# google-research/corenet

Hardware: AMD Instinct MI355X
Metric: voxels/sec fwd+bwd @128^3 (higher is better)
Workload: dtype bf16x3 (the convolutions of decoder stages 3-6 and the encoder's 3x3 convolutions -- forward of stages 4-5, data gradient of all -- multiply operands split into two bf16 terms: three bf16 MFMAs per product, fp32 accumulation, 16 mantissa bits, ~3e-6 relative per layer; tensors, everything else and t

## Files before the change

corenet_amd/_lib.py:

```python
from __future__ import annotations

import ctypes as C
import os
from typing import Optional

import torch as t

_HERE = os.path.dirname(os.path.abspath(__file__))
TOOLS_LIB_PATH = os.path.join(os.path.dirname(_HERE), "tools", "_build", "libcorenet_hip_tools.so")
PROBE_LIB_PATH = os.path.join(os.path.dirname(_HERE), "tools", "_build", "libcrn_probe.so")
LIB_PATH = os.environ.get("CORENET_HIP_LIB", TOOLS_LIB_PATH if os.environ.get("CRN_TOOLS_LIB") == "1" else
                          os.path.join(_HERE, "lib", "libcorenet_hip.so"))

c_i32p = C.POINTER(C.c_int32)
c_f32p = C.c_void_p
vp = C.c_void_p
i64 = C.c_int64
i32 = C.c_int
f32 = C.c_float
sz = C.c_size_t


class CrnTapBoxes(C.Structure):
  _fields_ = [("n_groups", C.c_int32), ("c_groups", C.c_int32), ("n_box", (C.c_int8 * 6) * 8),
# ... 53 lines not shown
                         C.POINTER(CrnView), i32, i32, i32, i32, i32, i32, i32, vp, vp],
    "crn_conv_fwd_bf3_slabs": [C.POINTER(CrnView), C.POINTER(CrnInTransform), vp, i32, vp, i32,
                               C.POINTER(CrnView), i32, i32, i32, i32, i32, i32, i32, vp, vp],
    "crn_conv_fwd_bf3_slabs_bnbwd": [C.POINTER(CrnView), C.POINTER(CrnInTransform), vp, i32, vp, i32,
                                     C.POINTER(CrnView), i32, i32, i32, i32, i32, i32, i32, vp, C.POINTER(CrnBnBwdFuse), vp],
    "crn_conv_fwd_bf3_slabs_stats": [C.POINTER(CrnView), C.POINTER(CrnInTransform), vp, i32, vp, i32,
                                     C.POINTER(CrnView), i32, i32, i32, i32, i32, i32, i32, vp, i32, vp, sz, C.POINTER(C.c_int), vp],
    "crn_batch_renorm_bwd_apply": [vp, i64, vp, i64, i32, i32, i64, i32, vp, vp, vp, vp, vp, i64, vp, vp, i32, vp, i32,
                                   vp, sz, i32, vp],
    "crn_conv_wgrad_bf3": [C.POINTER(CrnView), C.POINTER(CrnInTransform), C.POINTER(CrnView), vp, i32,
                           i32, i32, i32, i32, i32, i32, i32, vp],
    "crn_conv_wgrad_bf3_boxes": [C.POINTER(CrnView), C.POINTER(CrnInTransform), C.POINTER(CrnView), vp, i32,
                                 i32, i32, i32, i32, i32, i32, i32, vp, vp],
    "crn_conv_fwd_bf3_plan": [C.POINTER(CrnView), C.POINTER(CrnInTransform), vp, vp, i32, vp, i32,
                              C.POINTER(CrnView), i32, i32, i32, i32, i32, i32, i32, vp, vp, vp],
    "crn_conv_wgrad_bf3_plan": [C.POINTER(CrnView), C.POINTER(CrnInTransform), C.POINTER(CrnView), vp, i32,
                                i32, i32, i32, i32, i32, i32, i32, vp, vp],
    "crn_conv_wgrad": [C.POINTER(CrnView), C.POINTER(CrnInTransform), C.POINTER(CrnView), vp, i32,
                       i32, i32, i32, i32, i32, i32, i32, vp, vp],
    "crn_bf3_operands": [vp, vp, i32, i64, vp, vp],
    "crn_bf3_gather_image": [vp, vp, i32, vp, vp],
    "crn_convt_s2k7_fwd_bf3": [vp, i64, i32, i32, i32, i32, C.POINTER(CrnInTransform), vp, vp, vp, i64, i64, i32, vp],
    "crn_convt_s2k7_dgrad_bf3": [vp, i64, i64, i32, i32, i32, i32, i32, vp, vp, i64, i32, vp],
    "crn_convt_s2k7_c2_fwd_bf3": [vp, i64, i32, i32, i32, i32, C.POINTER(CrnInTransform), vp, vp, vp, i64, i64, i32, vp],
    "crn_convt_s2k7_c2_dgrad_bf3": [vp, i64, i64, i32, i32, i32, i32, i32, vp, vp, i64, i32, vp],
    "crn_convt_s2k7_wgrad_bf3": [vp, i64, i32, i32, i32, i32, C.POINTER(CrnInTransform), vp, i64, i64, i32, vp, i32, i32, vp, vp],
    "crn_convt_s2k7_ximage": [vp, i64, i32, i32, i32, i32, C.POINTER(CrnInTransform), vp, sz, vp],
    "crn_splitk_defer": [i32],
    "crn_splitk_reserve": [i64, vp],
    "crn_splitk_release": [vp],
    "crn_set_deterministic": [i32],
    "crn_roctx_push": [C.c_char_p],
    "crn_roctx_pop": [],
    "crn_comm_unique_id": [vp],
    "crn_comm_init": [vp, i32, i32, C.POINTER(vp)],
    "crn_comm_destroy": [vp],
    "crn_comm_info": [vp, C.POINTER(i32), C.POINTER(i32), C.POINTER(i32)],
    "crn_allreduce_f32": [vp, vp, i64, vp],
    "crn_broadcast_f32": [vp, vp, i64, i32, vp],
    "crn_conv_wgrad_1x1_bf3": [C.POINTER(CrnView), C.POINTER(CrnInTransform), C.POINTER(CrnView), vp, i32, i32, vp],
    "crn_conv_wgrad_2d_bf3": [C.POINTER(CrnView), C.POINTER(CrnInTransform), C.POINTER(CrnView), vp, i32, i32, i32, i32,
                              i32, i32, vp],
    "crn_conv2d_bf3": [C.POINTER(CrnView), C.POINTER(CrnInTransform), vp, i32, vp, i32, C.POINTER(CrnView),
                       i32, i32, i32, i32, i32, vp],
    "crn_conv2d_bf3_plan": [C.POINTER(CrnView), C.POINTER(CrnInTransform), vp, i32, vp, i32, C.POINTER(CrnView),
                            i32, i32, i32, i32, i32, vp],
    "crn_conv_wgrad_2d_bf3_plan": [C.POINTER(CrnView), C.POINTER(CrnInTransform), C.POINTER(CrnView), vp, i32, i32, i32, i32,
                                   i32, i32, vp],
    "crn_copy_tiles_f32": [vp, vp, vp, vp, vp, i64, i32, vp],
    "crn_copy_mats_f32": [vp, vp, vp, i64, i32, vp],
    "crn_gather_f32": [vp, vp, vp, i64, vp],
    "crn_scatter_f32": [vp, vp, vp, i64, i32, vp],
    "crn_bias_grad": [vp, i32, i32, i64, i64, vp, i32, vp, sz, vp],
    "crn_batch_renorm_stats": [vp, i32, i32, i64, i64, i32, vp, vp, vp, vp, vp, f32, f32, i32,
                               vp, vp, vp, vp, sz, vp],
    "crn_batch_renorm_stats_tail": [vp, i32, i32, i64, i64, vp, vp, vp, vp, vp, f32, f32, i32, vp, vp, vp, vp, sz,
                                    vp, vp, vp, i64, vp, i64, vp, i64, i32, vp, i32, vp],
    "crn_batch_renorm_bwd_head": [vp, i64, vp, i64, vp, i64, vp, i64, vp, i64, i32, i32, i64, vp, vp, vp, vp, vp, i64,
                                  vp, vp, i32, vp, i32, vp, sz, vp, i32, vp],
    "crn_batch_renorm_bwd": [vp, i64, vp, i64, i32, i32, i64, i32, i32, vp, vp, vp, vp, vp, i64,
                             vp, vp, i32, vp, i32, vp, sz, vp],
    "crn_affine_add_relu": [vp, vp, vp, vp, vp, vp, i32, i32, i64, i64, i64, vp, i64, vp, i64, i32, vp],
    "crn_relu_bwd_add": [vp, vp, vp, i32, i32, i64, i64, i64, i64, vp, i64, vp],
    "crn_preprocess_caffe": [vp, i32, i32, i32, vp, vp],
    "crn_stem_conv_fwd": [vp, i32, i32, i32, vp, vp, vp, vp, sz, vp],
    "crn_stem_conv_wgrad": [vp, i32, i32, i32, vp, vp, vp],
    "crn_batch_renorm_finalize": [vp, i32, i32, C.c_double, vp, vp, vp, vp, vp, f32, f32, vp, vp, vp, vp],
    "crn_bn_relu_maxpool_fwd": [vp, vp, vp, i32, i32, i32, i32, vp, vp, vp],
    "crn_bn_relu_maxpool_bwd": [vp, vp, i32, i32, i32, i32, vp, vp],
    "crn_relu_mean_fwd": [vp, i32, i32, i64, i64, vp, vp],
    "crn_relu_mean_bwd": [vp, vp, i32, i32, i64, i64, vp, i64, i32, vp],
    "crn_linear_fwd": [vp, vp, vp, i32, i32, i32, vp, i32, vp],
    "crn_linear_bwd": [vp, vp, vp, i32, i32, i32, i32, vp, vp, vp, vp],
    "crn_stride2_gather": [vp, vp, i32, i32, i32, i32, i32, i32, vp],
    "crn_stride2_scatter": [vp, vp, i32, i32, i32, i32, i32, i32, vp],
    "crn_fill_offset_channels": [vp, i32, i64, i64, i32, vp, vp],
    "crn_decoder_inputs": [vp, vp, i32, i32, C.POINTER(C.c_float), vp, vp, vp],
    "crn_ray_sample_fwd": [vp, i64, i64, i64, i32, i32, i32, i32, vp, vp, vp, i64, i32, i32, i32, vp],
    "crn_ray_sample_bwd": [vp, i64, i32, i32, i32, i32, i32, vp, vp, vp, i64, i32, i32, i32, vp],
    "crn_ray_sample_fwd_idx": [vp, i64, i64, i64, i32, i32, i32, i32, vp, vp, vp, i64, i32, i32, i32, vp, vp],
    "crn_ray_project": [vp, vp, i32, i32, i32, i32, i32, i32, vp, vp],
    "crn_ray_sample_bwd_idx": [vp, i64, i32, i32, i32, i32, i32, vp, vp, i64, i32, i32, i32, vp],
    "crn_loss_fwd_bwd": [i32, vp, vp, vp, i32, i32, i64, vp, vp, f32, vp, sz, vp],
    "crn_argmax_confusion": [vp, vp, i32, i32, i64, vp, vp, vp],
    "crn_softmax_superres": [vp, i32, i32, i32, i32, i32, i32, vp, vp],
    "crn_eval_labels": [vp, vp, vp, i32, i32, i32, i32, i32, i32, i32, i32, vp, vp, vp, vp],
    "crn_eval_labels_cpu": [vp, vp, vp, i32, i32, i32, i32, i32, i32, i32, i32, vp, vp, vp, i32],
    "crn_eval_scores_tiles": [vp],
    "crn_eval_scores": [vp, i32, vp, vp, i32, i32, i32, i32, i32, i32, i32, i32, i32, vp, vp, vp, vp],
    "crn_eval_scores_cpu": [vp, i32, vp, vp, i32, i32, i32, i32, i32, i32, i32, i32, i32, vp, vp, vp, i32],
    "crn_score_softmax": [vp, i32, i32, i64, vp, vp],
    "crn_score_softmax_cpu": [vp, i32, i32, i64, vp, i32],
    "crn_adam_step": [vp, vp, vp, vp, i64, f32, f32, f32, f32, f32, i32, vp],
    "crn_adam_set_hyper": [vp, f32, f32, f32, f32, f32, i32, vp],
    "crn_adam_step_hyper": [vp, vp, vp, vp, i64, vp, vp],
    "crn_fill_voxels": [vp, vp, i32, i32, i32, i32, i32, vp, sz, vp],
    "crn_fill_voxels_strided": [vp, C.POINTER(i64), vp, C.POINTER(i64), i32, i32, i32, i32, i32, vp, sz, vp],
    "crn_fill_voxels_cpu": [vp, vp, i32, i32, i32, i32, i32, i32],
    "crn_marching_cubes_count": [vp, C.POINTER(i64), i32, i32, i32, i32, f32, vp, sz, vp, vp],
    "crn_marching_cubes_emit": [vp, C.POINTER(i64), i32, i32, i32, i32, f32, vp, vp, sz, vp, vp, vp, vp],
    "crn_marching_cubes_cpu": [vp, C.POINTER(i64), i32, i32, i32, i32, f32, vp, vp, vp, vp, vp, i32],
    "crn_box_filter": [vp, C.POINTER(i64), vp, i32, i32, i32, i32, i32, vp, sz, vp],
    "crn_box_filter_cpu": [vp, C.POINTER(i64), vp, i32, i32, i32, i32, i32, i32],
    "crn_render_bin": [vp, vp, i32, i32, i32, i32, i64, vp, vp, vp, vp],
    "crn_render_raster": [vp, vp, vp, vp, i32, vp, i32, i32, i32, i32, vp, vp, vp, vp, vp, vp],
    "crn_render_cpu": [vp, vp, vp, vp, i32, vp, i32, i32, i32, vp, i32],
    "crn_render_raster_tex": [vp, vp, vp, vp, i32, vp, i32, i32, i32, i32, vp, vp, vp, vp, vp, vp, vp, vp, i32, i32, i32, vp],
    "crn_render_cpu_tex": [vp, vp, vp, vp, i32, vp, i32, i32, i32, vp, vp, vp, vp, i32, i32, i32, i32],
    "crn_render_raster_geometry": [vp, vp, i32, i32, i32, i32, vp, vp, vp, vp, vp, vp, vp, vp, vp],
    "crn_render_cpu_geometry": [vp, vp, i32, i32, i32, vp, vp, vp, vp, i32],
    "crn_voxel_faces_count": [vp, i32, i32, i32, i32, vp, i32, vp, vp, vp, sz, vp, vp],
    "crn_voxel_faces_emit": [vp, i32, i32, i32, i32, vp, i32, vp, i32, vp, sz, vp, vp, vp, vp],
    "crn_voxel_faces_cpu": [vp, i32, i32, i32, i32, vp, i32, vp, vp, vp, i32, vp, vp, vp, vp, i32],
    "crn_sample_surface": [vp, vp, i32, i64, i64, C.c_uint32, vp, sz, vp, vp, vp, vp],
    "crn_sample_surface_cpu": [vp, vp, i32, i64, C.c_uint32, vp, vp, vp, i32],
    "crn_nearest": [vp, vp, vp, vp, i32, i64, i64, i64, vp, sz, vp, vp, vp],
    "crn_nearest_cpu": [vp, vp, vp, vp, i32, vp, vp, i32],
    "crn_point_triangle": [vp, vp, vp, vp, i32, i64, i64, i64, i64, vp, sz, vp, vp, vp],
    "crn_point_triangle_cpu": [vp, vp, vp, vp, i32, vp, vp, i32],
    "crn_voxel_components_bricks": [vp],
    "crn_voxel_components": [vp, C.POINTER(i64), i32, i32, i32, i32, i32, i32, i32, vp, sz, vp, vp, vp],
    "crn_component_stats": [vp, vp, C.POINTER(i64), i32, i32, i32, i32, i32, vp, i64, vp, vp, vp, vp, vp],
    "crn_voxel_components_cpu": [vp, C.POINTER(i64), i32, i32, i32, i32, i32, i32, i32, vp, vp, i32],
    "crn_component_stats_cpu": [vp, vp, C.POINTER(i64), i32, i32, i32, i32, i32, vp, i64, vp, vp, vp, vp, i32],
    "crn_voxel_distance_tiles": [vp],
    "crn_voxel_distance": [vp, C.POINTER(i64), i32, i32, i32, i32, i32, i32, vp, sz, vp, vp, vp],
    "crn_voxel_distance_cpu": [vp, C.POINTER(i64), i32, i32, i32, i32, i32, i32, vp, vp, i32],
    "crn_voxel_visibility_tiles": [vp],
    "crn_voxel_visibility": [vp, C.POINTER(i64), i32, i32, i32, i32, i32, vp, i32, vp, sz, vp, vp, vp],
    "crn_voxel_visibility_cpu": [vp, C.POINTER(i64), i32, i32, i32, i32, i32, vp, i32, vp, vp, i32],
    "crn_voxel_overlap_tiles": [vp],
    "crn_voxel_overlap": [vp, C.POINTER(i64), i32, vp, C.POINTER(i64), i32, i32, i32, i32, i32, vp, vp, vp, vp, sz, vp, vp],
    "crn_voxel_overlap_cpu": [vp, C.POINTER(i64), i32, vp, C.POINTER(i64), i32, i32, i32, i32, i32, vp, vp, vp, vp, vp, i32],
    "crn_voxel_topology_tiles": [vp],
    "crn_voxel_topology": [vp, C.POINTER(i64), i32, i32, i32, i32, i32, i32, i32, vp, vp, vp],
    "crn_voxel_topology_cpu": [vp, C.POINTER(i64), i32, i32, i32, i32, i32, i32, i32, vp, vp, i32],
    "crn_mesh_tiles": [vp],
    "crn_mesh_corner_count": [vp, i64, vp, vp, i32, i64, vp, vp, vp],
    "crn_mesh_corner_lists": [vp, i64, vp, vp, i32, i64, vp, vp, vp, vp, vp, vp, vp, vp, vp],
    "crn_mesh_neighbours": [vp, vp, vp, i64, vp, vp],
    "crn_mesh_smooth_step": [vp, vp, vp, vp, vp, f32, i64, vp],
    "crn_mesh_face_normals": [vp, vp, i64, vp, vp, i32, i64, vp, vp],
    "crn_mesh_vertex_normals": [vp, vp, i64, vp, i32, i64, vp, vp, vp, vp],
    "crn_mesh_cluster_build": [vp, i64, vp, i64, vp, vp, i32, f32, vp, vp, i32, vp, vp, vp, vp, vp],
    "crn_mesh_cluster_emit": [vp, i64, vp, i64, vp, vp, i32, f32, vp, vp, vp, vp, vp, vp, vp, i64, i64, vp, vp, vp, vp, vp, vp],
    "crn_mesh_topology_cpu": [vp, i64, vp, vp, i32, i64, vp, vp, vp, vp, vp, vp],
    "crn_mesh_smooth_step_cpu": [vp, vp, vp, vp, vp, f32, i64],
    "crn_mesh_face_normals_cpu": [vp, vp, i64, vp, vp, i32, i64, vp],
    "crn_mesh_vertex_normals_cpu": [vp, vp, i64, vp, i32, i64, vp, vp, vp],
    "crn_mesh_cluster_cpu": [vp, i64, vp, i64, vp, vp, i32, f32, vp, vp, vp, vp, vp],
    "crn_voxelize_mesh": [vp, vp, i32, vp, i32, i32, i32, i32, i32, f32, i32, i32, vp, vp],
    "crn_batch_renorm_eval_affine": [vp, vp, vp, i32, f32, vp, vp, vp],
    "crn_transform_meshes": [vp, vp, i32, vp, i32, vp, vp],
    "crn_merge_labels": [vp, vp, vp, i32, i32, i32, i32, i32, vp, vp],
    "crn_zero_f32": [vp, i64, vp],
    "crn_add_i64": [vp, i32, i64, vp],
}
_SIZE_FNS = {
    "crn_batch_renorm_workspace_bytes": [i32],
    "crn_loss_workspace_bytes": [i32, i32],
    "crn_fill_voxels_workspace_bytes": [i32, i32, i32, i32],
    "crn_marching_cubes_workspace_bytes": [i32, i32, i32, i32],
    "crn_voxel_faces_workspace_bytes": [i32, i32, i32, i32],
    "crn_sample_surface_workspace_bytes": [i64, i32],
    "crn_nearest_workspace_bytes": [i64],
    "crn_point_triangle_workspace_bytes": [i64, i64],
# ... 130 lines not shown
```

corenet_amd/backend.py:

```python
from __future__ import annotations

import ctypes as C
from typing import Optional

import torch as t

from corenet_amd import _lib
from corenet_amd._lib import CrnInTransform, CrnView, ptr
from corenet_amd.views import View, space_to_depth_view, view_of

_DTYPE_CODE = {t.float32: 0, t.uint8: 1, t.int32: 2, t.float64: 3, t.int64: 4, t.int16: 5, t.int8: 6}


def _cview(v: View) -> CrnView:
  base = v.storage.data_ptr() + 4 * (v.offset - v.storage.storage_offset())
  c = v.__dict__.get("_crn")
  if c is None or c[0] != base:
    c = (base, CrnView(base, v.B, v.C, v.D, v.H, v.W, v.sB, v.sC, ptr(v.chan_off), v.sD, v.sH, v.sW))
    object.__setattr__(v, "_crn", c)
  return c[1]


class Transform:
  __slots__ = ("scale", "shift", "pre_relu", "post_relu")
# ... 279 lines not shown

  def bn_stats(self, x: t.Tensor, B, Cn, S, sB, pre_relu, gamma, beta, rmean, rvar, nbt, eps,
               momentum, training, scale, shift, saved):
    ws, n = self._bn_ws(Cn, x.device)
    self.lib.crn_batch_renorm_stats(ptr(x), B, Cn, S, sB, int(pre_relu), ptr(gamma), ptr(beta),
                                    ptr(rmean), ptr(rvar), ptr(nbt), eps, momentum, int(training),
                                    ptr(scale), ptr(shift), ptr(saved), ptr(ws), n, _lib.stream())

  def stem_conv_fwd(self, img: t.Tensor, w_packed: t.Tensor, bias, y: t.Tensor, stats: bool) -> int:
    B, _, H, W = img.shape
    parts = int(self.lib.crn_stem_conv_parts(B, H, W)) if stats else 0
    ws, n = self._bn_ws(64, img.device) if stats else (None, 0)
    self.lib.crn_stem_conv_fwd(ptr(img), B, H, W, ptr(w_packed), ptr(bias), ptr(y), ptr(ws), n, _lib.stream())
    return parts

  def bn_finalize(self, parts: int, Cn: int, count: float, gamma, beta, rmean, rvar, nbt, eps, momentum, scale, shift, saved):
    ws, _ = self._bn_ws(Cn, scale.device)
    self.lib.crn_batch_renorm_finalize(ptr(ws), parts, Cn, float(count), ptr(gamma), ptr(beta), ptr(rmean), ptr(rvar),
                                       ptr(nbt), eps, momentum, ptr(scale), ptr(shift), ptr(saved), _lib.stream())

  def bn_stats_tail(self, x, B, Cn, S, sB, gamma, beta, rmean, rvar, nbt, eps, momentum, training, scale, shift, saved,
                    r, rscale, rshift, sB_r, y_pre, sB_pre, y, sB_y, relu, y2=None, W=0):
    ws, n = self._bn_ws(Cn, x.device)
    self.lib.crn_batch_renorm_stats_tail(ptr(x), B, Cn, S, sB, ptr(gamma), ptr(beta), ptr(rmean), ptr(rvar), ptr(nbt),
                                         eps, momentum, int(training), ptr(scale), ptr(shift), ptr(saved), ptr(ws), n,
                                         ptr(r), ptr(rscale), ptr(rshift), sB_r, ptr(y_pre), sB_pre, ptr(y), sB_y,
                                         int(relu), ptr(y2), int(W), _lib.stream())

  def bn_bwd(self, x, sB_x, dy, sB_dy, B, Cn, S, pre_relu, post_relu, gamma, scale, shift, saved,
             dx, sB_dx, dgamma, dbeta, accumulate=False, dsum=None, ndsum=0):
    ws, n = self._bn_ws(Cn, x.device)
    self.lib.crn_batch_renorm_bwd(ptr(x), sB_x, ptr(dy), sB_dy, B, Cn, S, int(pre_relu),
                                  int(post_relu), ptr(gamma), ptr(scale), ptr(shift), ptr(saved),
                                  ptr(dx), sB_dx, ptr(dgamma), ptr(dbeta), int(accumulate),
                                  ptr(dsum), int(ndsum), ptr(ws), n, _lib.stream())

  def bn_bwd_head(self, x, sB_x, dy, sB_dy, g, sB_g, act, sB_act, g2, sB_g2, B, Cn, S, gamma, scale, shift, saved,
                  dx, sB_dx, dgamma, dbeta, accumulate=False, dsum=None, ndsum=0, g_compact=None, W=0):
    ws, n = self._bn_ws(Cn, x.device)
    self.lib.crn_batch_renorm_bwd_head(ptr(x), sB_x, ptr(dy), sB_dy, ptr(g), sB_g, ptr(act), sB_act, ptr(g2), sB_g2,
                                       B, Cn, S, ptr(gamma), ptr(scale), ptr(shift), ptr(saved), ptr(dx), sB_dx,
                                       ptr(dgamma), ptr(dbeta), int(accumulate), ptr(dsum), int(ndsum), ptr(ws), n,
                                       ptr(g_compact), int(W), _lib.stream())

  def bn_eval_affine(self, params, buffers, table, eps, scale, shift):
    self.lib.crn_batch_renorm_eval_affine(ptr(params), ptr(buffers), ptr(table), table.shape[0], eps,
                                          ptr(scale), ptr(shift), _lib.stream())

  def affine_add_relu(self, x, scale, shift, r, rscale, rshift, B, Cn, S, sB_x, sB_r,
                      y_pre, sB_pre, y, sB_y, relu):
    self.lib.crn_affine_add_relu(ptr(x), ptr(scale), ptr(shift), ptr(r), ptr(rscale), ptr(rshift),
                                 B, Cn, S, sB_x, sB_r, ptr(y_pre), sB_pre, ptr(y), sB_y, int(relu),
                                 _lib.stream())

  def relu_bwd_add(self, dy, y_pre, dy2, B, Cn, S, sB_dy, sB_pre, sB_dy2, dx, sB_dx):
    self.lib.crn_relu_bwd_add(ptr(dy), ptr(y_pre), ptr(dy2), B, Cn, S, sB_dy, sB_pre, sB_dy2,
                              ptr(dx), sB_dx, _lib.stream())

  def preprocess(self, img_u8, out):
    B, _, H, W = img_u8.shape
    self.lib.crn_preprocess_caffe(ptr(img_u8), B, H, W, ptr(out), _lib.stream())

  def maxpool_fwd(self, x, scale, shift, B, Cn, H, W, y, argmax):
    self.lib.crn_bn_relu_maxpool_fwd(ptr(x), ptr(scale), ptr(shift), B, Cn, H, W, ptr(y), ptr(argmax),
                                     _lib.stream())

  def maxpool_bwd(self, dy, argmax, B, Cn, H, W, dx):
    self.lib.crn_bn_relu_maxpool_bwd(ptr(dy), ptr(argmax), B, Cn, H, W, ptr(dx), _lib.stream())

  def relu_mean_fwd(self, x_pre, B, Cn, S, sB, avg):
    self.lib.crn_relu_mean_fwd(ptr(x_pre), B, Cn, S, sB, ptr(avg), _lib.stream())

  def relu_mean_bwd(self, x_pre, davg, B, Cn, S, sB, dx, sB_dx, accumulate=False):
    self.lib.crn_relu_mean_bwd(ptr(x_pre), ptr(davg), B, Cn, S, sB, ptr(dx), sB_dx, int(accumulate),
                               _lib.stream())

  def linear_fwd(self, x, w, bias, B, K, N, y, ldy):
    self.lib.crn_linear_fwd(ptr(x), ptr(w), ptr(bias), B, K, N, ptr(y), ldy, _lib.stream())

  def linear_bwd(self, x, w, dy, lddy, B, K, N, dx, dw, db):
    self.lib.crn_linear_bwd(ptr(x), ptr(w), ptr(dy), lddy, B, K, N, ptr(dx), ptr(dw), ptr(db),
                            _lib.stream())

  def stride2_gather(self, x, y):
    B, Cn, h, w = y.shape
    self.lib.crn_stride2_gather(ptr(x), ptr(y), B, Cn, h, w, x.shape[2], x.shape[3], _lib.stream())

  def stride2_scatter(self, dy, dx):
    B, Cn, h, w = dy.shape
    self.lib.crn_stride2_scatter(ptr(dy), ptr(dx), B, Cn, h, w, dx.shape[2], dx.shape[3], _lib.stream())

  def decoder_inputs(self, v2s, offset, scales, layer_mats, offset_out):
    n = len(scales)
    arr = (C.c_float * n)(*[float(v) for v in scales])
    self.lib.crn_decoder_inputs(ptr(v2s), ptr(offset), v2s.shape[0], n, arr, ptr(layer_mats), ptr(offset_out), _lib.stream())

  def fill_offset_channels(self, x, B, sB, S, c0, offset):
    self.lib.crn_fill_offset_channels(ptr(x), B, sB, S, c0, ptr(offset), _lib.stream())

  def ray_sample_fwd(self, fmap, map_sB, B, Cn, h, w, matrix, offset, out, out_sB, D, H, W,
                     map_sC=None, map_sP=1):
    self.lib.crn_ray_sample_fwd(ptr(fmap), map_sB, h * w if map_sC is None else map_sC, map_sP, B, Cn, h, w,
                                ptr(matrix), ptr(offset), ptr(out), out_sB, D, H, W, _lib.stream())

  def ray_sample_bwd(self, dout, dout_sB, B, Cn, D, H, W, matrix, offset, dmap, dmap_sB, h, w,
                     zero_first=True):
    self.lib.crn_ray_sample_bwd(ptr(dout), dout_sB, B, Cn, D, H, W, ptr(matrix), ptr(offset),
                                ptr(dmap), dmap_sB, h, w, int(zero_first), _lib.stream())

  def ray_sample_fwd_idx(self, fmap, map_sB, B, Cn, h, w, matrix, offset, out, out_sB, D, H, W, idx,
                         map_sC=None, map_sP=1):
    self.lib.crn_ray_sample_fwd_idx(ptr(fmap), map_sB, h * w if map_sC is None else map_sC, map_sP, B, Cn, h, w,
                                    ptr(matrix), ptr(offset), ptr(out), out_sB, D, H, W, ptr(idx), _lib.stream())

  def ray_project(self, matrix, offset, B, D, H, W, h, w, idx):
    self.lib.crn_ray_project(ptr(matrix), ptr(offset), B, D, H, W, h, w, ptr(idx), _lib.stream())

  def ray_sample_bwd_idx(self, dout, dout_sB, B, Cn, D, H, W, idx, dmap, dmap_sB, h, w, zero_first=True):
    self.lib.crn_ray_sample_bwd_idx(ptr(dout), dout_sB, B, Cn, D, H, W, ptr(idx), ptr(dmap), dmap_sB, h, w,
                                    int(zero_first), _lib.stream())

  def loss_fwd_bwd(self, kind, logits, gt_i32, B, Cn, S, loss, dlogits, grad_scale=1.0, weights=None):
    n = self.lib.crn_loss_workspace_bytes(B, Cn)
    ws = self.workspace("loss", n, logits.device)
    self.lib.crn_loss_fwd_bwd(kind, ptr(logits), ptr(gt_i32), ptr(weights), B, Cn, S, ptr(loss), ptr(dlogits),
                              grad_scale, ptr(ws), n, _lib.stream())

  def loss_labels_in_range(self, B, Cn, device) -> bool:
    n = self.lib.crn_loss_workspace_bytes(B, Cn)
    ws = self.workspace("loss", n, device)
    off = self.lib.crn_loss_status_ptr(ptr(ws), B) - ws.data_ptr()
    return int(ws[off:off + 4].view(t.int32)) == 0

  def loss_partials(self, B, Cn, S, device) -> t.Tensor:
    ws = self.workspace("loss", self.lib.crn_loss_workspace_bytes(B, Cn), device)
    nblk = min(max(1, -(-S // 2048)), 512)
    return ws[:B * nblk * 48].view(t.float64).view(B, nblk, 6).clone()

  def softmax_superres(self, logits, m, B, Cn, D, H, W, out):
    self.lib.crn_softmax_superres(ptr(logits), m, B, Cn, D, H, W, ptr(out), _lib.stream())

  def argmax_confusion(self, logits, gt_i32, B, Cn, S, labels, cm):
    self.lib.crn_argmax_confusion(ptr(logits), ptr(gt_i32), B, Cn, S, ptr(labels), ptr(cm), _lib.stream())

  def eval_labels(self, scores, gt_i32, scene_class, B, Cn, K, D, H, W, m, n, labels, cm, bad):
    self.lib.crn_eval_labels(ptr(scores), ptr(gt_i32), ptr(scene_class), B, Cn, K, D, H, W, m, n, ptr(labels), ptr(cm), ptr(bad),
                             _lib.stream())

  def eval_scores(self, scores, from_logits, gt_i32, scene_class, B, Cn, K, D, H, W, m, n, nbins, table, sq, bad):
    self.lib.crn_eval_scores(ptr(scores), int(bool(from_logits)), ptr(gt_i32), ptr(scene_class), B, Cn, K, D, H, W, m, n, nbins,
                             ptr(table), ptr(sq), ptr(bad), _lib.stream())

  def score_softmax(self, logits, B, Cn, S, out):
    self.lib.crn_score_softmax(ptr(logits), B, Cn, S, ptr(out), _lib.stream())

  def adam_step(self, p, g, m, v, n, lr, b1, b2, eps, grad_scale, step):
    self.lib.crn_adam_step(ptr(p), ptr(g), ptr(m), ptr(v), n, lr, b1, b2, eps, grad_scale, step,
                           _lib.stream())

  def adam_set_hyper(self, hyper, lr, b1, b2, eps, grad_scale, step):
    self.lib.crn_adam_set_hyper(ptr(hyper), lr, b1, b2, eps, grad_scale, step, _lib.stream())

  def adam_step_hyper(self, p, g, m, v, n, hyper):
    self.lib.crn_adam_step_hyper(ptr(p), ptr(g), ptr(m), ptr(v), n, ptr(hyper), _lib.stream())

  def add_i64(self, p, n, v):
    self.lib.crn_add_i64(ptr(p), n, v, _lib.stream())

  def zero(self, x: t.Tensor):
    self.lib.crn_zero_f32(ptr(x), x.numel(), _lib.stream())

  def fill_voxels(self, grid: t.Tensor, out: t.Tensor):
    N, D, H, W = grid.shape
    n = self.lib.crn_fill_voxels_workspace_bytes(N, D, H, W)
    ws = self.workspace("fill", n, grid.device)
    if grid.is_contiguous() and out.is_contiguous():
      self.lib.crn_fill_voxels(ptr(grid), ptr(out), _DTYPE_CODE[grid.dtype], N, D, H, W, ptr(ws), n,
                               _lib.stream())
    else:
      gs = (C.c_int64 * 4)(*grid.stride())
      os_ = (C.c_int64 * 4)(*out.stride())
      self.lib.crn_fill_voxels_strided(ptr(grid), gs, ptr(out), os_, _DTYPE_CODE[grid.dtype], N, D, H, W,
                                       ptr(ws), n, _lib.stream())

  def marching_cubes_count(self, grid: t.Tensor, level: float, counts: t.Tensor):
    N, D, H, W = grid.shape
    n = self.lib.crn_marching_cubes_workspace_bytes(N, D, H, W)
    ws = self.workspace("mc", n, grid.device)
    st = (C.c_int64 * 4)(*grid.stride())
    self.lib.crn_marching_cubes_count(ptr(grid), st, N, D, H, W, float(level), ptr(ws), n, ptr(counts), _lib.stream())

  def marching_cubes_emit(self, grid: t.Tensor, level: float, matrices: Optional[t.Tensor], vertices: t.Tensor,
                          normals: t.Tensor, faces: t.Tensor):
    N, D, H, W = grid.shape
    n = self.lib.crn_marching_cubes_workspace_bytes(N, D, H, W)
    ws = self.workspace("mc", n, grid.device)
    st = (C.c_int64 * 4)(*grid.stride())
    self.lib.crn_marching_cubes_emit(ptr(grid), st, N, D, H, W, float(level), ptr(matrices), ptr(ws), n, ptr(vertices),
                                     ptr(normals), ptr(faces), _lib.stream())

  def box_filter(self, grid: t.Tensor, k: int, out: t.Tensor):
    N, D, H, W = grid.shape
    n = 4 * grid.numel()
    ws = self.workspace("box", n, grid.device)
    st = (C.c_int64 * 4)(*grid.stride())
    self.lib.crn_box_filter(ptr(grid), st, ptr(out), N, D, H, W, int(k), ptr(ws), n, _lib.stream())

  def voxel_components(self, grid: t.Tensor, connectivity: int, by_value: bool, labels: t.Tensor, num: t.Tensor):
    N, D, H, W = grid.shape
# ... 127 lines not shown
```

corenet_amd/csrc/batch_renorm.hip:

```cpp
#include "crn_common.h"
#include <cstdlib>
#include <algorithm>
#include <type_traits>

namespace {

constexpr int kThreads = 256;

struct Slice { int64_t s0, s1; };
__device__ __forceinline__ Slice block_slice(int64_t S) {
  int64_t chunk = (S + gridDim.x - 1) / gridDim.x;
  chunk = (chunk + 3) & ~(int64_t)3;
  Slice r;
  r.s0 = (int64_t)blockIdx.x * chunk;
  r.s1 = min(S, r.s0 + chunk);
  return r;
}

template <bool VEC, typename F4, typename F1>
__device__ __forceinline__ void for_slice(Slice sl, F4 f4, F1 f1) {
  if (VEC) {
#pragma unroll 4
    for (int64_t s = sl.s0 + (int64_t)threadIdx.x * 4; s + 3 < sl.s1; s += (int64_t)kThreads * 4) f4(s);
    const int64_t nfull = (sl.s1 > sl.s0) ? ((sl.s1 - sl.s0) & ~(int64_t)3) : 0;
// ... 442 lines not shown
  crn_block_sum2(p1, p2, redd, s1, s2);
  if (threadIdx.x == 0) {
    const BnAffineGrad ag = bn_bwd_close(s1, s2, count, saved[2 * C + c], saved[3 * C + c], sm);
    if (blockIdx.x == 0 && b == 0) bn_bwd_store_grad(ag, c, dgamma, dbeta, accumulate);
  }
  __syncthreads();
  const float mg = sm[0], mgx = sm[1];
  const float* px = x + (int64_t)b * sBx + (int64_t)c * S;
  const float* pg = dy + (int64_t)b * sBdy + (int64_t)c * S;
  float* po = dx + (int64_t)b * sBdx + (int64_t)c * S;
  float lsum = 0.f;
  auto one = [&](float xr, float gv) -> float {
    const float o = bn_bwd_dx(xr, gv, pre_relu, post_relu, ch, k, mg, mgx);
    lsum += o;
    return o;
  };
  for_slice<VEC>(block_slice(S),
                 [&](int64_t s) { const f32x4 a = *reinterpret_cast<const f32x4*>(px + s);
                                  const f32x4 g = *reinterpret_cast<const f32x4*>(pg + s);
                                  f32x4 o; o.x = one(a.x, g.x); o.y = one(a.y, g.y);
                                  o.z = one(a.z, g.z); o.w = one(a.w, g.w);
                                  *reinterpret_cast<f32x4*>(po + s) = o; },
                 [&](int64_t s) { po[s] = one(px[s], pg[s]); });
  if (dsum && c < ndsum) {
    const float tsum = bn_block_sum_f32(lsum, red);
    if (threadIdx.x == 0) atomicAdd(dsum + c, tsum);
  }
}

template <bool VEC>
__global__ __launch_bounds__(kThreads) void bn_owner_bwd_kernel(
    const float* x, int64_t sBx, const float* dy, int64_t sBdy, int B, int64_t S, int C, int pre_relu,
    int post_relu, const float* gamma, const float* scale, const float* shift, const float* saved, float* dx,
    int64_t sBdx, float* dgamma, float* dbeta, int accumulate, float* dsum, int ndsum) {
  __shared__ double red[kThreads / 64];
  __shared__ float sm[2];
  __shared__ float redf[kThreads / 64];
  const int c = blockIdx.x;
  const BnBwdChannel ch = bn_bwd_channel(c, C, scale, shift, saved);
  Slice all; all.s0 = 0; all.s1 = S;
  double s1 = 0.0, s2 = 0.0;
  auto acc = [&](float xv, float gv) { bn_bwd_acc(xv, gv, pre_relu, post_relu, ch, s1, s2); };
  for (int b = 0; b < B; ++b) {
    const float* px = x + (int64_t)b * sBx + (int64_t)c * S;
    const float* pg = dy + (int64_t)b * sBdy + (int64_t)c * S;
    for_slice<VEC>(all,
                   [&](int64_t s) { const f32x4 a = *reinterpret_cast<const f32x4*>(px + s);
                                    const f32x4 g = *reinterpret_cast<const f32x4*>(pg + s);
                                    acc(a.x, g.x); acc(a.y, g.y); acc(a.z, g.z); acc(a.w, g.w); },
                   [&](int64_t s) { acc(px[s], pg[s]); });
  }
  const double t1 = crn_block_sum(s1, red);
  const double t2 = crn_block_sum(s2, red);
  if (threadIdx.x == 0)
    bn_bwd_store_grad(bn_bwd_close(t1, t2, (double)B * (double)S, saved[2 * C + c], saved[3 * C + c], sm), c, dgamma, dbeta,
                      accumulate);
  __syncthreads();
  const float mg = sm[0], mgx = sm[1];
  const float k = gamma[c] * saved[2 * C + c] * ch.rstd;
  float lsum = 0.f;
  auto one = [&](float xr, float gv) -> float {
    const float o = bn_bwd_dx(xr, gv, pre_relu, post_relu, ch, k, mg, mgx);
    lsum += o;
    return o;
  };
  for (int b = 0; b < B; ++b) {
    const float* px = x + (int64_t)b * sBx + (int64_t)c * S;
    const float* pg = dy + (int64_t)b * sBdy + (int64_t)c * S;
    float* po = dx + (int64_t)b * sBdx + (int64_t)c * S;
    for_slice<VEC>(all,
                   [&](int64_t s) { const f32x4 a = *reinterpret_cast<const f32x4*>(px + s);
                                    const f32x4 g = *reinterpret_cast<const f32x4*>(pg + s);
                                    f32x4 o; o.x = one(a.x, g.x); o.y = one(a.y, g.y);
                                    o.z = one(a.z, g.z); o.w = one(a.w, g.w);
                                    *reinterpret_cast<f32x4*>(po + s) = o; },
                   [&](int64_t s) { po[s] = one(px[s], pg[s]); });
  }
  if (dsum && c < ndsum) {
    const float tsum = bn_block_sum_f32(lsum, redf);
    if (threadIdx.x == 0) dsum[c] = tsum;
  }
}

inline bool owner_form(int64_t S, int C, int B) {
  return C >= 64 && (int64_t)B * S <= 65536 && ((int64_t)B * S <= 16384 || C >= 256);
}

template <bool VEC>
__global__ __launch_bounds__(kThreads) void affine_add_relu_kernel(
    const float* x, const float* scale, const float* shift, const float* r, const float* rscale,
    const float* rshift, int64_t S, int64_t sBx, int64_t sBr, float* y_pre, int64_t sBpre,
    float* y, int64_t sBy, int relu) {
  crn_kernargs_now(x, scale, shift, r, rscale, rshift, S, sBx, sBr, y_pre, sBpre, y, sBy, relu);
  const int c = blockIdx.y, b = blockIdx.z;
  const float sc = scale ? scale[c] : 1.f, sh = shift ? shift[c] : 0.f;
  const float rsc = rscale ? rscale[c] : 1.f, rsh = rshift ? rshift[c] : 0.f;
  const float* px = x + (int64_t)b * sBx + (int64_t)c * S;
  const float* pr = r ? r + (int64_t)b * sBr + (int64_t)c * S : nullptr;
  float* pp = y_pre ? y_pre + (int64_t)b * sBpre + (int64_t)c * S : nullptr;
  float* py = y ? y + (int64_t)b * sBy + (int64_t)c * S : nullptr;
  auto one = [&](float xv, float rv) -> float { return xv * sc + sh + (pr ? rv * rsc + rsh : 0.f); };
  for_slice<VEC>(block_slice(S),
                 [&](int64_t s) {
                   const f32x4 a = *reinterpret_cast<const f32x4*>(px + s);
                   f32x4 q = (f32x4){0.f, 0.f, 0.f, 0.f};
                   if (pr) q = *reinterpret_cast<const f32x4*>(pr + s);
                   f32x4 o; o.x = one(a.x, q.x); o.y = one(a.y, q.y); o.z = one(a.z, q.z); o.w = one(a.w, q.w);
                   if (pp) *reinterpret_cast<f32x4*>(pp + s) = o;
                   if (py) {
                     if (relu) { o.x = fmaxf(o.x, 0.f); o.y = fmaxf(o.y, 0.f); o.z = fmaxf(o.z, 0.f); o.w = fmaxf(o.w, 0.f); }
                     *reinterpret_cast<f32x4*>(py + s) = o;
                   }
                 },
                 [&](int64_t s) {
                   const float o = one(px[s], pr ? pr[s] : 0.f);
                   if (pp) pp[s] = o;
                   if (py) py[s] = relu ? fmaxf(o, 0.f) : o;
                 });
}

template <bool VEC>
__global__ __launch_bounds__(kThreads) void relu_bwd_add_kernel(
    const float* dy, const float* y_pre, const float* dy2, int64_t S, int64_t sBdy, int64_t sBpre,
    int64_t sBdy2, float* dx, int64_t sBdx) {
  crn_kernargs_now(dy, y_pre, dy2, S, sBdy, sBpre, sBdy2, dx, sBdx);
  const int c = blockIdx.y, b = blockIdx.z;
  const float* pg = dy ? dy + (int64_t)b * sBdy + (int64_t)c * S : nullptr;
  const float* pp = y_pre + (int64_t)b * sBpre + (int64_t)c * S;
  const float* p2 = dy2 ? dy2 + (int64_t)b * sBdy2 + (int64_t)c * S : nullptr;
  float* po = dx + (int64_t)b * sBdx + (int64_t)c * S;
  auto one = [&](float g, float p, float g2) -> float { return (p > 0.f ? g : 0.f) + g2; };
  for_slice<VEC>(block_slice(S),
                 [&](int64_t s) {
                   f32x4 g = (f32x4){0.f, 0.f, 0.f, 0.f}, g2 = g;
                   if (pg) g = *reinterpret_cast<const f32x4*>(pg + s);
                   const f32x4 p = *reinterpret_cast<const f32x4*>(pp + s);
                   if (p2) g2 = *reinterpret_cast<const f32x4*>(p2 + s);
                   f32x4 o; o.x = one(g.x, p.x, g2.x); o.y = one(g.y, p.y, g2.y);
                   o.z = one(g.z, p.z, g2.z); o.w = one(g.w, p.w, g2.w);
                   *reinterpret_cast<f32x4*>(po + s) = o;
                 },
                 [&](int64_t s) { po[s] = one(pg ? pg[s] : 0.f, pp[s], p2 ? p2[s] : 0.f); });
}

template <bool VEC>
__global__ __launch_bounds__(kThreads) void bias_grad_partial_kernel(const float* dy, int64_t S,
                                                                      int64_t sB, double* ws) {
  __shared__ double red[kThreads / 64];
  const int c = blockIdx.y, b = blockIdx.z;
  const float* p = dy + (int64_t)b * sB + (int64_t)c * S;
  double s1 = 0.0;
  for_slice<VEC>(block_slice(S),
                 [&](int64_t s) { const f32x4 v = *reinterpret_cast<const f32x4*>(p + s);
                                  s1 += (double)v.x + (double)v.y + (double)v.z + (double)v.w; },
                 [&](int64_t s) { s1 += (double)p[s]; });
  const double t1 = crn_block_sum(s1, red);
  if (threadIdx.x == 0) {
    const int nparts = gridDim.x * gridDim.z;
    ws[(int64_t)c * nparts + (int64_t)b * gridDim.x + blockIdx.x] = t1;
  }
}

__global__ __launch_bounds__(kThreads) void bias_grad_owner_kernel(const float* dy, int B, int64_t S, int64_t sB,
                                                                    float* db, int accumulate) {
  __shared__ double red[kThreads / 64];
  crn_kernargs_now(dy, B, S, sB, db, accumulate);
// ... 312 lines not shown
  float* const dsum_det = (dsum && ndsum > 0 && crn_deterministic()) ? dsum : nullptr;
  if (dsum_det && ws_bytes < (size_t)ndsum * ns * B * sizeof(double)) return CRN_ENOMEM;
  { const int rcf = crn_splitk_flush(st); if (rcf != CRN_OK) return rcf; }
  dim3 grid(ns, C, B);
  if (dsum_det) dsum = nullptr;
  with_bool(vec_ok(S, {sB_x, sB_dy, sB_dx}, {x, dy, dx}), [&](auto vec) {
    hipLaunchKernelGGL(bn_bwd_apply_kernel<decltype(vec)::value>, grid, dim3(kThreads), 0, st, x, sB_x, dy, sB_dy, S, C,
                       pre_relu, 0, gamma, scale, shift, saved, ws, nparts,
                       (double)B * (double)S, dx, sB_dx, dgamma, dbeta, accumulate, dsum, ndsum);
  });
  CRN_CHECK_LAUNCH();
  if (dsum_det) return bias_grad_ordered(dx, B, ndsum, S, sB_dx, ns, dsum_det, 0, ws, ws_bytes, st);
  return CRN_OK;
}

extern "C" int crn_batch_renorm_bwd_head(const float* x, int64_t sB_x, float* dy, int64_t sB_dy,
                                         const float* g, int64_t sB_g, const float* act, int64_t sB_act,
                                         const float* g2, int64_t sB_g2,
                                         int B, int C, int64_t S, const float* gamma, const float* scale,
                                         const float* shift, const float* saved, float* dx, int64_t sB_dx,
                                         float* dgamma, float* dbeta, int accumulate, float* dsum, int ndsum,
                                         double* ws, size_t ws_bytes, const float* g_compact, int W, crnStream stream) {
  if (!g || !act || !dy) return CRN_EINVAL;
  if (g_compact && (W < 1 || S % W || sB_g != (int64_t)C * S)) return CRN_EINVAL;
  const int H = g_compact ? (int)(S / W) : 0, H2 = (H + 1) / 2, W2 = (W + 1) / 2;
  const BnHead head{g, sB_g, act, sB_act, g2, sB_g2, g_compact, (int64_t)C * H2 * W2, W, W2, H2};
  return bn_bwd_impl(x, sB_x, dy, sB_dy, B, C, S, 0, 0, gamma, scale, shift, saved, dx, sB_dx, dgamma, dbeta,
                     accumulate, dsum, ndsum, ws, ws_bytes, stream, &head);
}

extern "C" int crn_affine_add_relu(const float* x, const float* scale, const float* shift,
                                   const float* r, const float* rscale, const float* rshift,
                                   int B, int C, int64_t S, int64_t sB_x, int64_t sB_r,
                                   float* y_pre, int64_t sB_pre, float* y, int64_t sB_y, int relu,
                                   crnStream stream) {
  CRN_ENTRY(stream);
  return crn_affine_add_relu_impl(x, scale, shift, r, rscale, rshift, B, C, S, sB_x, sB_r, y_pre, sB_pre, y, sB_y, relu, stream);
}
int crn_affine_add_relu_impl(const float* x, const float* scale, const float* shift, const float* r, const float* rscale,
                             const float* rshift, int B, int C, int64_t S, int64_t sB_x, int64_t sB_r, float* y_pre,
                             int64_t sB_pre, float* y, int64_t sB_y, int relu, crnStream stream) {
  hipStream_t st = (hipStream_t)stream;
  if (B < 1 || C < 1 || S < 1 || (!y && !y_pre)) return CRN_EINVAL;
  dim3 grid(nsplit_for(S, C, B), C, B);
  with_bool(vec_ok(S, {sB_x, r ? sB_r : 0, y_pre ? sB_pre : 0, y ? sB_y : 0}, {x, r, y_pre, y}), [&](auto vec) {
    hipLaunchKernelGGL(affine_add_relu_kernel<decltype(vec)::value>, grid, dim3(kThreads), 0, st, x, scale, shift, r, rscale,
                       rshift, S, sB_x, sB_r, y_pre, sB_pre, y, sB_y, relu);
  });
  CRN_CHECK_LAUNCH();
  return CRN_OK;
}

extern "C" int crn_relu_bwd_add(const float* dy, const float* y_pre, const float* dy2, int B, int C,
                                int64_t S, int64_t sB_dy, int64_t sB_pre, int64_t sB_dy2, float* dx,
                                int64_t sB_dx, crnStream stream) {
  CRN_ENTRY(stream);
  return crn_relu_bwd_add_impl(dy, y_pre, dy2, B, C, S, sB_dy, sB_pre, sB_dy2, dx, sB_dx, stream);
}
int crn_relu_bwd_add_impl(const float* dy, const float* y_pre, const float* dy2, int B, int C, int64_t S, int64_t sB_dy,
                          int64_t sB_pre, int64_t sB_dy2, float* dx, int64_t sB_dx, crnStream stream) {
  hipStream_t st = (hipStream_t)stream;
  if (B < 1 || C < 1 || S < 1 || !y_pre || !dx) return CRN_EINVAL;
  dim3 grid(nsplit_for(S, C, B), C, B);
  with_bool(vec_ok(S, {dy ? sB_dy : 0, sB_pre, dy2 ? sB_dy2 : 0, sB_dx}, {dy, y_pre, dy2, dx}), [&](auto vec) {
    hipLaunchKernelGGL(relu_bwd_add_kernel<decltype(vec)::value>, grid, dim3(kThreads), 0, st, dy, y_pre, dy2, S, sB_dy,
                       sB_pre, sB_dy2, dx, sB_dx);
  });
  CRN_CHECK_LAUNCH();
  return CRN_OK;
}

extern "C" int crn_bias_grad(const float* dy, int B, int C, int64_t S, int64_t sB, float* db,
                             int accumulate, double* ws, size_t ws_bytes, crnStream stream) {
  CRN_ENTRY(stream);
  hipStream_t st = (hipStream_t)stream;
  if (B < 1 || C < 1 || S < 1 || B > 64) return CRN_EINVAL;
  if ((int64_t)B * S <= 65536) {
    hipLaunchKernelGGL(bias_grad_owner_kernel, dim3(C), dim3(kThreads), 0, st, dy, B, S, sB, db, accumulate);
    CRN_CHECK_LAUNCH();
    return CRN_OK;
  }
  return bias_grad_ordered(dy, B, C, S, sB, nsplit_for(S, C, B), db, accumulate, ws, ws_bytes, st);
}
```

corenet_amd/csrc/losses.hip:

```cpp
#include "crn_common.h"
#include <algorithm>
#include <cmath>

namespace {

constexpr int kThreads = 256;
constexpr int kNQ = 6;

template <int CT>
struct Soft {
  float s[CT];
  float logz;
  __device__ __forceinline__ void compute(const float* l, int64_t S, int C) {
    float m = -INFINITY;
#pragma unroll
    for (int c = 0; c < CT; ++c) { s[c] = c < C ? l[c * S] : -INFINITY; m = fmaxf(m, s[c]); }
    float z = 0.f;
#pragma unroll
    for (int c = 0; c < CT; ++c) { s[c] = c < C ? expf(s[c] - m) : 0.f; z += s[c]; }
    const float inv = 1.0f / z;
#pragma unroll
    for (int c = 0; c < CT; ++c) s[c] *= inv;
    logz = m + logf(z);
  }
};

template <int CT>
__global__ __launch_bounds__(kThreads) void loss_pass1_kernel(const float* logits, const int32_t* gt,
                                                              const float* weights, int C, int64_t S, double* part) {
  __shared__ double red[kThreads / 64];
  const int b = blockIdx.y;
  const float* lb = logits + (int64_t)b * C * S;
  const int32_t* gb = gt + (int64_t)b * S;
  const float* wb = weights ? weights + (int64_t)b * S : nullptr;
  double q[kNQ] = {0, 0, 0, 0, 0, 0};
  for (int64_t v = blockIdx.x * (int64_t)kThreads + threadIdx.x; v < S; v += (int64_t)gridDim.x * kThreads) {
    Soft<CT> sm;
    sm.compute(lb + v, S, C);
    int g = gb[v];
    if (g < 0 || g >= C) { q[5] += 1.0; g = 0; }
    const float w = wb ? wb[v] : 1.f;
    float pfg = 0.f;
#pragma unroll
    for (int c = 1; c < CT; ++c) pfg += sm.s[c];
    const float gf = g >= 1 ? 1.f : 0.f;
    q[0] += (double)(fminf(gf, pfg) * w);
    q[1] += (double)(fmaxf(gf, pfg) * w);
    float ia = 0.f, ua = 0.f;
#pragma unroll
    for (int c = 1; c < CT; ++c) {
      if (c < C) {
        if (c == g) { ia += sm.s[c] * ((float)(C - 1) * w); ua += (float)(C - 1) * w; }
        else ua += sm.s[c] * w;
      }
    }
    q[2] += (double)ia; q[3] += (double)ua;
    q[4] += (double)((sm.logz - lb[v + (int64_t)g * S]) * w);
  }
  for (int k = 0; k < kNQ; ++k) {
    const double t = crn_block_sum(q[k], red);
    if (threadIdx.x == 0) part[((int64_t)b * gridDim.x + blockIdx.x) * kNQ + k] = t;
  }
}

__global__ __launch_bounds__(1024) void loss_finalize_kernel(const double* part, int nblk, int B, int64_t S, int kind,
                                                            float grad_scale, float* loss, float* coef, int* bad_label) {
  __shared__ double sums[64 * kNQ];
  const int lane = threadIdx.x & 63, wave = threadIdx.x >> 6;
  for (int pair = wave; pair < B * kNQ; pair += (int)(blockDim.x >> 6)) {
    const int b = pair / kNQ, k = pair - b * kNQ;
    double s = 0.0;
    for (int i = lane; i < nblk; i += 64) s += part[((int64_t)b * nblk + i) * kNQ + k];
    s = crn_wave_sum(s);
    if (lane == 0) sums[pair] = s;
  }
  __syncthreads();
  if (threadIdx.x != 0) return;
  double iou_fg = 0.0, iou_ag = 0.0, xs = 0.0, nbad = 0.0;
  for (int b = 0; b < B; ++b) {
    const double* q = sums + b * kNQ;
    nbad += q[5];
    const float ifg = (float)q[0], ufg = (float)q[1] == 0.f ? 1.f : (float)q[1];
    const float iag = (float)q[2], uag = (float)q[3] == 0.f ? 1.f : (float)q[3];
    iou_fg += (double)(ifg / ufg); iou_ag += (double)(iag / uag);
    xs += q[4];
    coef[4 + b * 4 + 0] = ifg; coef[4 + b * 4 + 1] = ufg; coef[4 + b * 4 + 2] = iag; coef[4 + b * 4 + 3] = uag;
  }
  const float Lfg = 1.f - (float)(iou_fg / B), Lag = 1.f - (float)(iou_ag / B);
  const float X = (float)(xs / ((double)B * (double)S));
  float L = 0.f, kfg = 0.f, kag = 0.f, kx = 0.f;
  switch (kind) {
    case 0: L = Lfg; kfg = 1.f; break;
    case 1: L = (1.f + Lag) * (1.f + X); kag = 1.f + X; kx = 1.f + Lag; break;
    case 2: L = Lag; kag = 1.f; break;
    case 3: L = X; kx = 1.f; break;
    case 4: L = (1.f + Lfg) * (1.f + X); kfg = 1.f + X; kx = 1.f + Lfg; break;
  }
  *bad_label = nbad > 0.0 ? 1 : 0;
  loss[0] = L;
  coef[0] = L; coef[1] = kfg * grad_scale / B; coef[2] = kag * grad_scale / B;
  coef[3] = kx * grad_scale / (float)((double)B * (double)S);
}

template <int CT>
__global__ __launch_bounds__(kThreads) void loss_pass2_kernel(const float* logits, const int32_t* gt,
                                                              const float* weights, int C, int64_t S,
                                                              const float* coef, float* dlogits) {
  const int b = blockIdx.y;
  const float* lb = logits + (int64_t)b * C * S;
  const int32_t* gb = gt + (int64_t)b * S;
  const float* wb = weights ? weights + (int64_t)b * S : nullptr;
  float* db = dlogits + (int64_t)b * C * S;
  const float kfg0 = coef[1], kag0 = coef[2], kx0 = coef[3];
  const float ifg = coef[4 + b * 4 + 0], ufg = coef[4 + b * 4 + 1];
  const float iag = coef[4 + b * 4 + 2], uag = coef[4 + b * 4 + 3];
  for (int64_t v = blockIdx.x * (int64_t)kThreads + threadIdx.x; v < S; v += (int64_t)gridDim.x * kThreads) {
    Soft<CT> sm;
    sm.compute(lb + v, S, C);
    int g = gb[v];
    if (g < 0 || g >= C) g = 0;
    const float w = wb ? wb[v] : 1.f;
    const float kfg = kfg0 * w, kag = kag0 * w, kx = kx0 * w;
    float d[CT];
#pragma unroll
    for (int c = 0; c < CT; ++c) d[c] = 0.f;
    if (kfg0 != 0.f) {
      float pfg = 0.f;
#pragma unroll
      for (int c = 1; c < CT; ++c) pfg += sm.s[c];
      const float dp = g >= 1 ? -kfg / ufg : kfg * ifg / (ufg * ufg);
#pragma unroll
      for (int c = 0; c < CT; ++c) d[c] += dp * sm.s[c] * ((c >= 1 ? 1.f : 0.f) - pfg);
    }
    if (kag0 != 0.f) {
      float qv[CT];
      float dot = 0.f;
#pragma unroll
      for (int c = 0; c < CT; ++c) {
        qv[c] = 0.f;
        if (c >= 1 && c < C) qv[c] = (c == g) ? -kag * (float)(C - 1) / uag : kag * iag / (uag * uag);
        dot += qv[c] * sm.s[c];
      }
#pragma unroll
      for (int c = 0; c < CT; ++c) d[c] += sm.s[c] * (qv[c] - dot);
    }
    if (kx0 != 0.f) {
#pragma unroll
      for (int c = 0; c < CT; ++c) d[c] += kx * (sm.s[c] - (c == g ? 1.f : 0.f));
    }
#pragma unroll
    for (int c = 0; c < CT; ++c)
      if (c < C) db[v + (int64_t)c * S] = d[c];
  }
}

template <int CT>
__global__ __launch_bounds__(kThreads) void argmax_confusion_kernel(const float* logits, const int32_t* gt,
                                                                    int C, int64_t S, int32_t* labels,
                                                                    unsigned long long* cm) {
  extern __shared__ int hist[];
  for (int i = threadIdx.x; i < C * C; i += kThreads) hist[i] = 0;
  __syncthreads();
  const int b = blockIdx.y;
  const float* lb = logits + (int64_t)b * C * S;
  for (int64_t v = blockIdx.x * (int64_t)kThreads + threadIdx.x; v < S; v += (int64_t)gridDim.x * kThreads) {
    float best = lb[v];
    int bi = 0;
#pragma unroll
    for (int c = 1; c < CT; ++c)
      if (c < C) { const float x = lb[v + (int64_t)c * S]; if (x > best) { best = x; bi = c; } }
    if (labels) labels[(int64_t)b * S + v] = bi;
    if (gt) {
      const int g = gt[(int64_t)b * S + v];
      if (g >= 0 && g < C) atomicAdd(&hist[g * C + bi], 1);
    }
  }
  __syncthreads();
  if (gt)
    for (int i = threadIdx.x; i < C * C; i += kThreads)
      if (hist[i]) atomicAdd(&cm[i], (unsigned long long)hist[i]);
}

inline int loss_nblk(int64_t S) { return (int)std::min<int64_t>(std::max<int64_t>(1, (S + kThreads * 8 - 1) / (kThreads * 8)), 512); }

}

extern "C" size_t crn_loss_workspace_bytes(int B, int C) {
  (void)C;
  return (size_t)B * 512 * kNQ * sizeof(double) + (size_t)(4 + 4 * B) * sizeof(float) + 64;
}

extern "C" int crn_loss_fwd_bwd(int kind, const float* logits, const int32_t* gt, const float* weights, int B, int C,
                                int64_t S, float* loss, float* dlogits, float grad_scale, void* workspace,
                                size_t workspace_bytes, crnStream stream) {
  CRN_ENTRY(stream);
  hipStream_t st = (hipStream_t)stream;
  if (kind < 0 || kind > 4 || B < 1 || B > 64 || C < 2 || C > 32 || S < 1 || !logits || !gt || !loss) return CRN_EINVAL;
  if (workspace_bytes < crn_loss_workspace_bytes(B, C)) return CRN_ENOMEM;
  const int nblk = loss_nblk(S);
  double* part = reinterpret_cast<double*>(workspace);
  float* coef = reinterpret_cast<float*>(part + (size_t)B * 512 * kNQ);
  int* bad_label = reinterpret_cast<int*>(coef + 4 + 4 * B + (16 - (4 + 4 * B) % 16) % 16);
  dim3 grid(nblk, B);
#define CRN_LOSS_P1(CT) hipLaunchKernelGGL(loss_pass1_kernel<CT>, grid, dim3(kThreads), 0, st, logits, gt, weights, C, S, part)
  if (C <= 2) CRN_LOSS_P1(2); else if (C <= 4) CRN_LOSS_P1(4); else if (C <= 8) CRN_LOSS_P1(8);
  else if (C <= 16) CRN_LOSS_P1(16); else CRN_LOSS_P1(32);
#undef CRN_LOSS_P1
  CRN_CHECK_LAUNCH();
  hipLaunchKernelGGL(loss_finalize_kernel, dim3(1), dim3(1024), 0, st, part, nblk, B, S, kind, grad_scale, loss, coef, bad_label);
  CRN_CHECK_LAUNCH();
  if (dlogits) {
#define CRN_LOSS_P2(CT) hipLaunchKernelGGL(loss_pass2_kernel<CT>, grid, dim3(kThreads), 0, st, logits, gt, weights, C, S, coef, dlogits)
    if (C <= 2) CRN_LOSS_P2(2); else if (C <= 4) CRN_LOSS_P2(4); else if (C <= 8) CRN_LOSS_P2(8);
    else if (C <= 16) CRN_LOSS_P2(16); else CRN_LOSS_P2(32);
#undef CRN_LOSS_P2
    CRN_CHECK_LAUNCH();
  }
  return CRN_OK;
}

extern "C" const int* crn_loss_status_ptr(void* workspace, int B) {
  double* part = reinterpret_cast<double*>(workspace);
  float* coef = reinterpret_cast<float*>(part + (size_t)B * 512 * kNQ);
  return reinterpret_cast<int*>(coef + 4 + 4 * B + (16 - (4 + 4 * B) % 16) % 16);
}

extern "C" int crn_argmax_confusion(const float* logits, const int32_t* gt, int B, int C, int64_t S,
                                    int32_t* labels, int64_t* cm, crnStream stream) {
  CRN_ENTRY(stream);
  hipStream_t st = (hipStream_t)stream;
  if (B < 1 || C < 1 || C > 32 || S < 1 || !logits || (gt && !cm)) return CRN_EINVAL;
  dim3 grid(loss_nblk(S), B);
  const size_t sh = (size_t)C * C * sizeof(int);
#define CRN_AM(CT) hipLaunchKernelGGL(argmax_confusion_kernel<CT>, grid, dim3(kThreads), sh, st, logits, gt, C, S, labels, reinterpret_cast<unsigned long long*>(cm))
  if (C <= 2) CRN_AM(2); else if (C <= 4) CRN_AM(4); else if (C <= 8) CRN_AM(8);
  else if (C <= 16) CRN_AM(16); else CRN_AM(32);
#undef CRN_AM
  CRN_CHECK_LAUNCH();
  return CRN_OK;
}

namespace {
template <int CT>
__global__ __launch_bounds__(256) void softmax_superres_kernel(const float* __restrict__ logits, int m, int B, int C,
                                                               int D, int H, int W, float* __restrict__ out) {
  const int64_t So = (int64_t)D * m * H * m * W * m, S = (int64_t)D * H * W;
  const int b = blockIdx.y;
  for (int64_t o = blockIdx.x * (int64_t)blockDim.x + threadIdx.x; o < So; o += (int64_t)gridDim.x * blockDim.x) {
    const int Wo = W * m, Ho = H * m;
    const int X = (int)(o % Wo), Y = (int)((o / Wo) % Ho), Z = (int)(o / ((int64_t)Wo * Ho));
    const int n = ((Z % m) * m + (Y % m)) * m + (X % m);
    const int64_t s = ((int64_t)(Z / m) * H + (Y / m)) * W + (X / m);
    const float* src = logits + (((int64_t)n * B + b) * C) * S + s;
    float v[CT];
    float mx = -3.4e38f;
#pragma unroll
    for (int c = 0; c < CT; ++c) { v[c] = c < C ? src[(int64_t)c * S] : -3.4e38f; mx = fmaxf(mx, v[c]); }
    float sum = 0.f;
#pragma unroll
    for (int c = 0; c < CT; ++c) { v[c] = c < C ? expf(v[c] - mx) : 0.f; sum += v[c]; }
    float* dst = out + ((int64_t)b * C) * So + o;
#pragma unroll
    for (int c = 0; c < CT; ++c) if (c < C) dst[(int64_t)c * So] = v[c] / sum;
  }
}
}

extern "C" int crn_softmax_superres(const float* logits, int m, int B, int C, int D, int H, int W, float* out,
                                    crnStream stream) {
  CRN_ENTRY(stream);
  hipStream_t st = (hipStream_t)stream;
  if (!logits || !out || m < 1 || B < 1 || C < 1 || C > 32 || D < 1 || H < 1 || W < 1) return CRN_EINVAL;
  const int64_t So = (int64_t)D * H * W * m * m * m;
  dim3 grid((unsigned)std::min<int64_t>(crn_cdiv(So, 256), 65535), (unsigned)B);
#define CRN_SM(CT) hipLaunchKernelGGL(softmax_superres_kernel<CT>, grid, dim3(256), 0, st, logits, m, B, C, D, H, W, out)
  if (C <= 2) CRN_SM(2); else if (C <= 4) CRN_SM(4); else if (C <= 8) CRN_SM(8);
  else if (C <= 16) CRN_SM(16); else CRN_SM(32);
#undef CRN_SM
  CRN_CHECK_LAUNCH();
  return CRN_OK;
}
```

corenet_amd/model/core_net.py:

```python
from __future__ import annotations

import contextlib
import os
import sys
import dataclasses
import math
from typing import Any, Dict, Optional, Tuple

import torch as t
from torch import nn

from corenet_amd import _lib
from corenet_amd.model.engine import Engine, LOSS_KINDS, check_image_hw, on_stream


@dataclasses.dataclass(frozen=True)
class DecoderConfig:
  resolution: Tuple[int, int, int]
  num_output_channels: int
  last_upscale_factor: int = 2
  latent_channels: int = 64
  skip_fraction: float = 0.75


# ... 279 lines not shown
    B = image.shape[0]
    C = self.engine.num_classes
    D, H, W = plan.logits.shape[2:]
    with t.no_grad():
      stash = t.empty((n, B, C, D, H, W), dtype=plan.logits.dtype, device=plan.logits.device)
      for i in range(n):
        stash[i].copy_(plan.forward_decoder(v2s, offs[i], training=False))
      be = self.engine.be
      if m > 0:
        out = t.empty((B, C, m * D, m * H, m * W), dtype=stash.dtype, device=stash.device)
        be.softmax_superres(stash, m, B, C, D, H, W, out)
        return out
      out = t.empty_like(stash)
      be.softmax_superres(stash, 1, n * B, C, D, H, W, out)
      return out

  def multi_offset_labels(self, image: t.Tensor, voxel_projection_matrix: t.Tensor, grid_offsets: t.Tensor,
                          resolution_multiplier: int, gt: Optional[t.Tensor] = None, num_classes: Optional[int] = None,
                          scene_classes: Optional[t.Tensor] = None, cm: Optional[t.Tensor] = None,
                          bad: Optional[t.Tensor] = None) -> t.Tensor:
    m = int(resolution_multiplier)
    if m < 1:
      raise ValueError("resolution_multiplier >= 1 expected")
    if gt is not None and (cm is None or bad is None):
      raise ValueError("multi_offset_labels: cm and bad are required with gt")
    from corenet_amd import voxel_metrics
    B, C = image.shape[0], self.engine.num_classes
    D, H, W = self.engine.resolution
    K = voxel_metrics.check_eval_labels_args((B, C, D, H, W), image.device, gt, num_classes, scene_classes, m, None, cm, bad)
    plan, v2s, offs, n, m = self._multi_offset_encoder(image, voxel_projection_matrix, grid_offsets, m)
    assert plan.logits.shape == (B, C, D, H, W) and plan.logits.is_contiguous()
    labels = t.empty((B, m * D, m * H, m * W), dtype=t.int32, device=plan.logits.device)
    be = self.engine.be
    with t.no_grad():
      for i in range(n):
        logits = plan.forward_decoder(v2s, offs[i], training=False)
        be.eval_labels(logits, gt, scene_classes, B, C, K, D, H, W, m, i, labels, cm, bad)
    return labels

  def multi_offset_score_histogram(self, image: t.Tensor, voxel_projection_matrix: t.Tensor, grid_offsets: t.Tensor,
                                   resolution_multiplier: int, gt: t.Tensor, num_classes: Optional[int] = None,
                                   scene_classes: Optional[t.Tensor] = None, nbins: int = 20, out=None):
    m = int(resolution_multiplier)
    if m < 1:
      raise ValueError("resolution_multiplier >= 1 expected")
    from corenet_amd import score_metrics
    B, C = image.shape[0], self.engine.num_classes
    D, H, W = self.engine.resolution
    K = score_metrics.check_score_args((B, C, D, H, W), image.device, gt, num_classes, scene_classes, m, nbins, out)
    plan, v2s, offs, n, m = self._multi_offset_encoder(image, voxel_projection_matrix, grid_offsets, m)
    assert plan.logits.shape == (B, C, D, H, W) and plan.logits.is_contiguous()
    if out is None:
      out = score_metrics.empty_histogram(K, nbins, plan.logits.device)
    be = self.engine.be
    with t.no_grad():
      for i in range(n):
        logits = plan.forward_decoder(v2s, offs[i], training=False)
        be.eval_scores(logits, True, gt, scene_classes, B, C, K, D, H, W, m, i, int(nbins), out.table, out.sq, out.bad)
    return out

  def train_step(self, image: t.Tensor, voxel_projection_matrix: t.Tensor,
                 voxel_sample_locations: t.Tensor, grid: t.Tensor, loss: str = "iou_fgbg",
                 lr: float = 4e-4, adam_eps: float = 1e-4, world_size: int = 1,
                 all_reduce=None, graph: Optional[bool] = None) -> t.Tensor:
    eng = self.engine
    self._check_image(image)
    B, C = image.shape[0], eng.num_classes
    if tuple(grid.shape) != (B,) + tuple(eng.resolution):
      raise ValueError(f"grid of shape {tuple(grid.shape)}, expected {(B,) + tuple(eng.resolution)}")
    with self._on_device():
      plan = eng.plan(B, image.shape[2:])
      if all_reduce is not None and getattr(all_reduce, "needs_buffer_broadcast", False):
        all_reduce.broadcast_buffers_once()
      if graph is None:
        graph = os.environ.get("CRN_GRAPH", "0") == "1"
      if all_reduce is not None and hasattr(all_reduce, "_active") and not all_reduce._active():
        if hasattr(all_reduce, "pushed"):
          all_reduce.pushed.clear()
        all_reduce = None
      graphable = (all_reduce is None and eng.device.type == "cuda" and plan.probes is None and plan.trace is None)
      if graph and graphable:
        return self._train_step_graph(plan, image, voxel_projection_matrix, voxel_sample_locations, grid, loss, lr,
                                      adam_eps, 1.0 / world_size)
      plan.forward(image.contiguous(), voxel_projection_matrix, voxel_sample_locations, training=True)
      if grid.dtype == t.int32 and grid.device == plan.gt.device and grid.is_contiguous() and grid.shape == plan.gt.shape:
        gt = grid
      else:
        plan.gt.copy_(grid); gt = plan.gt
      eng.be.loss_fwd_bwd(LOSS_KINDS[loss], plan.logits, gt, B, C, plan.logits[0, 0].numel(), plan.loss,
                          plan.glogits, 1.0)
      if all_reduce is not None and getattr(all_reduce, "overlap", False):
        all_reduce.pushed.clear()
        step_buckets = hasattr(all_reduce, "opt_stream") and plan.overlap and all_reduce.opt_stream() is not None
        if step_buckets:
          ost = all_reduce.opt_stream()
          ost.wait_stream(t.cuda.current_stream())
          with on_stream(ost):
            eng.adam_step_graphable(lr, adam_eps, grad_scale=1.0 / world_size, launch=False)
          all_reduce.after_bucket = eng.adam_bucket_hook()
        plan.backward(plan.glogits, grad_hook=all_reduce.push)
        plan._probe("grad_exchange_wait", all_reduce.wait)
        if step_buckets:
          all_reduce.after_bucket = None
          eng.weights_dirty = True
          return plan.loss
      elif all_reduce is None and plan.overlap:
        with plan._on_side():
          eng.adam_step_graphable(lr, adam_eps, grad_scale=1.0 / world_size, launch=False)
        plan.backward(plan.glogits, grad_hook=eng.adam_bucket_hook())
        eng.weights_dirty = True
        return plan.loss
      else:
        plan.backward(plan.glogits)
        if all_reduce is not None:
          all_reduce(eng.store.grads)
      eng.adam_step(lr, adam_eps, grad_scale=1.0 / world_size)
      return plan.loss

  def _step_body(self, plan, loss: str):
    eng = self.engine
    eng.weights_dirty = True
    plan.forward(plan.in_image, plan.in_v2s, plan.in_off, training=True)
    eng.be.loss_fwd_bwd(LOSS_KINDS[loss], plan.logits, plan.gt, plan.B, eng.num_classes, plan.logits[0, 0].numel(),
                        plan.loss, plan.glogits, 1.0)
    plan.backward(plan.glogits)
    eng.adam_update_from_hyper()

  def _train_step_graph(self, plan, image, v2s, offset, grid, loss, lr, adam_eps, grad_scale) -> t.Tensor:
    eng = self.engine
    plan.in_image.copy_(image); plan.in_v2s.copy_(v2s); plan.in_off.copy_(offset); plan.gt.copy_(grid)
    eng.adam_step_graphable(lr, adam_eps, grad_scale=grad_scale, launch=False)
    g = plan.graphs.get(loss)
    if g is None and plan.eager_steps < 1:
      self._step_body(plan, loss)
      plan.eager_steps += 1
      return plan.loss
    if g is None:
      g = t.cuda.CUDAGraph()
      cap = eng.capture_stream()
      cap.wait_stream(t.cuda.current_stream())
      with t.cuda.graph(g, stream=cap), _lib.pinned_stream(cap):
        self._step_body(plan, loss)
      t.cuda.current_stream().wait_stream(cap)
      plan.graphs[loss] = g
      _LIVE_GRAPHS.append(g)
    g.replay()
    eng.weights_dirty = True
    return plan.loss
```

corenet_amd/model/engine.py:

```python
from __future__ import annotations

import dataclasses
import os
from typing import Dict, List, Optional, Tuple

import numpy as np
import torch as t

from corenet_amd import _lib
from corenet_amd import views as V
from corenet_amd.backend import Transform
from corenet_amd.model import conv_geometry as G

IMAGE_HW = (256, 256)


def check_image_hw(hw):
  H, W = int(hw[0]), int(hw[1])
  if H < 32 or W < 32 or H % 4 or W % 4 or H * W > 4096 * 4096:
    raise ValueError(f"corenet_amd.CoreNet: image batch of {H}x{W} pixels; this engine takes H and W that are multiples of 4 and >= 32 "
                     f"(256x256 in every shipped config)")
  return H, W
BN_EPS = 1e-3
BN_MOMENTUM = 0.01
# ... 110 lines not shown
  rvar: t.Tensor
  nbt: t.Tensor
  dgamma: t.Tensor
  dbeta: t.Tensor
  scale: t.Tensor
  shift: t.Tensor
  saved: t.Tensor


@dataclasses.dataclass
class Conv:
  name: str
  fwd: G.Geom
  dgrad: Optional[G.Geom]
  wf: t.Tensor
  wd: Optional[t.Tensor]
  bias: t.Tensor
  gwf: t.Tensor
  dbias: t.Tensor
  n_ref: int
  wop_f: Optional[t.Tensor] = None
  wop_d: Optional[t.Tensor] = None
  wop_kind: str = ""
  ct_f: Optional[t.Tensor] = None
  ct_d: Optional[t.Tensor] = None
  ct_kind: str = ""


@dataclasses.dataclass(slots=True, eq=False)
class EncBlock:
  prefix: str; stage: str; cin: int; f: Tuple[int, int, int]; stride: int; h: int; w: int
  down: bool
  final: bool
  ya: t.Tensor; yb: t.Tensor; yc: t.Tensor; ys: Optional[t.Tensor]; out: t.Tensor
  gpre: t.Tensor; gyc: t.Tensor; gab: t.Tensor; gyb: t.Tensor; gaa: t.Tensor; gya: t.Tensor
  gys: Optional[t.Tensor]; gin: Optional[t.Tensor]
  xs: Optional[t.Tensor]; gxs: Optional[t.Tensor]
  xs_next: Optional["EncBlock"] = None
  inp: Optional[t.Tensor] = None
  xs_filled: bool = False


@dataclasses.dataclass(slots=True, eq=False)
class DecStage:
  cin: int; cmid: int; cout: int; r: int
  u: t.Tensor; gu: t.Tensor; w: t.Tensor; gw: t.Tensor; gv1: t.Tensor; gv2: t.Tensor

  def __getitem__(self, field: str):
    return getattr(self, field)


class on_stream:
  __slots__ = ("stream", "after", "_torch", "_pin")

  def __init__(self, stream, after=None):
    self.stream, self.after = stream, after
    self._torch, self._pin = t.cuda.stream(stream), _lib.pinned_stream(stream)

  def __enter__(self):
    self._torch.__enter__(); self._pin.__enter__()
    if self.after is not None:
      self.stream.wait_event(self.after)

  def __exit__(self, *exc):
    self._pin.__exit__(*exc); self._torch.__exit__(*exc)


_NO_KW = {}
_ORPHANS = []


class Engine:

  def __init__(self, num_classes: int, resolution=(128, 128, 128), latent_channels: int = 64,
               skip_fraction: float = 0.75, last_upscale_factor: int = 2, device="cuda",
               backend=None, dtype=t.float32, decoder_math: Optional[str] = None):
    if tuple(resolution) != (128, 128, 128) or last_upscale_factor != 2:
      raise ValueError("the CoReNet decoder is only defined for resolution 128^3, "
                       "last_upscale_factor 2 (reconstruction_decoder.py:38-54,93-95)")
    if backend is None:
      from corenet_amd.backend import default_backend
      backend = default_backend()
    self.be = backend
    default_math = "bf16x3" if getattr(backend, "name", "") == "hip" else "fp32"
    self.decoder_math = decoder_math or os.environ.get("CRN_DECODER_MATH", default_math)
    if self.decoder_math not in ("fp32", "bf16x3"):
      raise ValueError(f"decoder_math must be 'fp32' or 'bf16x3', not {self.decoder_math!r}")
    self.encoder_e2d = self.decoder_math == "bf16x3"
    assert dtype == t.float32 or getattr(backend, "name", "") == "emu"
    self.dtype = dtype
    self.device = t.device(device)
    if self.device.type == "cuda" and self.device.index is None:
      self.device = t.device("cuda", t.cuda.current_device() if t.cuda.is_available() else 0)
    self.num_classes = num_classes
    self.latent = latent_channels
    self.resolution = tuple(resolution)
    self.specs = param_specs(num_classes, latent_channels, skip_fraction)
    self.store = ParamStore(self.specs, self.device, dtype)
    self.skip_ch = {2: round(128 * skip_fraction), 3: round(64 * skip_fraction),
                    4: round(32 * skip_fraction), 5: round(16 * skip_fraction)}
    self._build_layers()
    self.plans: Dict[int, "Plan"] = {}
    self.adam_m: Optional[t.Tensor] = None
    self.adam_v: Optional[t.Tensor] = None
    self.adam_t = 0
    self.adam_hyper: Optional[t.Tensor] = None
    self.dgrad_dirty = True
    self.weights_dirty = True
    self.exchange = None
    self._side = False
    self._capture = None
    self._pack_ev = self._dgrad_packed = self._dec_packed = self._enc_late_packed = None
    self._enc_late_pending = False
    self._dec_pack_pending = False
    self._dgrad_pack_pending = False
    self._gpacked_zeroed = False

  def orphan_graph_resources(self):
    graphs = [g for p in self.plans.values() for g in list(p.graphs.values()) + [p.eval_graph] if g is not None]
    for p in self.plans.values():
      p.graphs, p.eval_graph, p.eval_eager = {}, None, 0
    if graphs or self._capture is not None:
      _ORPHANS.append((self.be, graphs, self._capture))
    self._capture = None

  @staticmethod
  def drain_orphans():
    while _ORPHANS:
      be, graphs, stream = _ORPHANS.pop()
      for g in graphs:
        try:
          g.reset()
        except Exception:
          pass
      if stream is not None:
        be.splitk_release(stream)

  def capture_stream(self):
    Engine.drain_orphans()
    if self._capture is None:
      self._capture = t.cuda.Stream(device=self.device)
    self.be.splitk_reserve(self._capture, floats=0)
    return self._capture

  def release_graph_resources(self):
    for p in self.plans.values():
      for g in list(p.graphs.values()) + ([p.eval_graph] if p.eval_graph is not None else []):
        try:
          g.reset()
        except Exception:
          pass
      p.graphs, p.eval_graph, p.eval_eager = {}, None, 0
    if self._capture is not None:
      self.be.splitk_release(self._capture)
      self._capture = None

  def side_stream(self):
    if self._side is False:
      use = self.device.type == "cuda"
      self._side = t.cuda.Stream(device=self.device) if use else None
      if use:
        self._pack_ev, self._dgrad_packed = t.cuda.Event(), t.cuda.Event()
        self._dec_packed, self._enc_late_packed = t.cuda.Event(), t.cuda.Event()
    return self._side

  def _bn(self, prefix: str) -> BN:
# ... 205 lines not shown

  @property
  def weights_dirty(self) -> bool:
    return self._weights_dirty

  @weights_dirty.setter
  def weights_dirty(self, v: bool):
    self._weights_dirty = v
    if v:
      self.dgrad_dirty = True

  def pack_weights(self, part: str = "all"):
    tiles = {"all": self.pack_tiles, "enc": self.pack_tiles_enc, "dec": self.pack_tiles_dec,
             "enc_early": self.pack_tiles_enc_early, "enc_late": self.pack_tiles_enc_late}[part]
    self.be.copy_tiles(self.store.params, self.packed, tiles)
    self._operands(*{"all": ("enc_early", "enc_late", "dec"), "enc": ("enc_early", "enc_late"), "dec": ("dec",),
                     "enc_early": ("enc_early",), "enc_late": ("enc_late",)}[part])
    if part in ("all", "dec"):
      self._weights_dirty = False

  def pack_dgrad_weights(self):
    self.be.copy_tiles(self.store.params, self.packed, self.pack_tiles_bwd)
    self._operands("bwd")
    self.dgrad_dirty = False

  def plan(self, batch: int, hw=IMAGE_HW) -> "Plan":
    hw = (int(hw[0]), int(hw[1]))
    key = batch if hw == IMAGE_HW else (batch, hw[0], hw[1])
    p = self.plans.get(key)
    if p is None:
      p = Plan(self, batch, hw)
      self.plans[key] = p
    return p

  def adam_step(self, lr: float, eps: float, betas=(0.9, 0.999), grad_scale: float = 1.0):
    if self.adam_m is None:
      self.adam_m = t.zeros_like(self.store.params)
      self.adam_v = t.zeros_like(self.store.params)
    self.adam_t += 1
    self.be.adam_step(self.store.params, self.store.grads, self.adam_m, self.adam_v,
                      self.store.params.numel(), lr, betas[0], betas[1], eps, grad_scale, self.adam_t)
    self.weights_dirty = True

  def adam_step_graphable(self, lr: float, eps: float, betas=(0.9, 0.999), grad_scale: float = 1.0, launch: bool = True):
    if self.adam_m is None:
      self.adam_m = t.zeros_like(self.store.params)
      self.adam_v = t.zeros_like(self.store.params)
    if self.adam_hyper is None:
      self.adam_hyper = t.zeros(8, dtype=t.float32, device=self.device)
    self.adam_t += 1
    self.be.adam_set_hyper(self.adam_hyper, lr, betas[0], betas[1], eps, grad_scale, self.adam_t)
    if launch:
      self.adam_update_from_hyper()

  def adam_bucket_hook(self):
    def hook(gslice: t.Tensor):
      lo, n = gslice.storage_offset(), gslice.numel()
      self.be.adam_step_hyper(self.store.params[lo:lo + n], gslice, self.adam_m[lo:lo + n], self.adam_v[lo:lo + n], n,
                              self.adam_hyper)
    return hook

  def adam_update_from_hyper(self):
    self.be.adam_step_hyper(self.store.params, self.store.grads, self.adam_m, self.adam_v,
                            self.store.params.numel(), self.adam_hyper)
    self.weights_dirty = True


def _no_exchange(grads: t.Tensor):
  """Bucket hook of a step without a gradient exchange."""


class Plan:

  def __init__(self, eng: Engine, B: int, hw=IMAGE_HW):
    self.eng, self.B = eng, B
    H, W = check_image_hw(hw)
    self.hw = (H, W)
    self.stem_hw = (H // 2, W // 2)
    parts = int(eng.be.lib.crn_stem_conv_parts(B, H, W)) if hasattr(eng.be, "stem_conv_fwd") else 0
    self.stem_fast = 0 < parts <= 4096
    self.dec_stats_fused = hasattr(eng.be, "conv_fwd_stats")
    self.pool_hw = (H // 4, W // 4)
    self.be = eng.be
    self.generation = 0
    self.graphs = {}
    self.eager_steps = 0
    self.eval_graph = None
    self.eval_eager = 0
    self._views = {}
    dev = eng.device
    self.dev = dev
    f = lambda *shape: t.zeros(*shape, dtype=eng.dtype, device=dev)
    self.in_image = t.zeros(B, 3, H, W, dtype=t.uint8, device=dev)
    self.in_v2s = f(B, 4, 4)
    self.in_off = f(B, 3)
    self.img = f(B, 3, H, W)
    self.y1 = f(B, 64, *self.stem_hw)
    self.gy1 = f(B, 64, *self.stem_hw); self.gy1b = f(B, 64, *self.stem_hw)
    self.p1 = f(B, 64, *self.pool_hw)
    self.p1_arg = t.zeros(B, 64, *self.pool_hw, dtype=t.int32, device=dev)
    self.blocks = []
    cin, (hi, wi) = 64, self.pool_hw
    stage_hw = {}
    for name, blocks, filt, stride in ENC_STAGES:
      for bl in blocks:
        st = stride if bl == "a" else 1
        ho, wo = (hi + st - 1) // st, (wi + st - 1) // st
        z = lambda c: f(B, c, ho, wo)
        s2 = st == 2
        blk = EncBlock(prefix=f"encoder.{name}.{bl}.", stage=name, cin=cin, f=filt, stride=st, h=ho, w=wo, down=(bl == "a"),
                       final=(bl == blocks[-1]), ya=z(filt[0]), yb=z(filt[1]), yc=z(filt[2]), ys=z(filt[2]) if bl == "a" else None,
                       out=z(filt[2]), gpre=z(filt[2]), gyc=z(filt[2]), gab=z(filt[1]), gyb=z(filt[1]), gaa=z(filt[0]), gya=z(filt[0]),
                       gys=z(filt[2]) if bl == "a" else None, gin=f(B, cin, hi, wi) if bl == "a" else None,
                       xs=z(cin) if s2 else None, gxs=z(cin) if s2 else None)
        if s2 and self.blocks:
          self.blocks[-1].xs_next = blk
        self.blocks.append(blk)
        cin, hi, wi = filt[2], ho, wo
      stage_hw[name] = (hi, wi)
    self.stage_hw = stage_hw
    self.feat = {"stage2": f(B, 256 + 3, *stage_hw["stage2"]), "stage3": f(B, 512 + 3, *stage_hw["stage3"]),
                 "stage4": f(B, 1024 + 3, *stage_hw["stage4"]), "stage5": f(B, 2048 + 3, *stage_hw["stage5"])}
    self.gfeat = {k: t.zeros_like(v) for k, v in self.feat.items()}
    self.avg = f(B, 2048); self.gavg = f(B, 2048)
    L = eng.latent
    self.z0 = f(B, L + 3); self.gz0 = f(B, L + 3); self.gv0 = f(B, L + 3)
    C = eng.num_classes
    sk = eng.skip_ch
    self.dec = {}
    for k, (ci, cm, co, r) in {2: (256, 256, 128, 4), 3: (128 + sk[2], 128, 64, 8), 4: (64 + sk[3], 64, 32, 16),
                               5: (32 + sk[4], 32, 16, 32), 6: (16 + sk[5], 16, C, 64)}.items():
      self.dec[k] = DecStage(ci, cm, co, r, u=f(B, ci, r, r, r), gu=f(B, ci, r, r, r), w=f(B, cm, r, r, r), gw=f(B, cm, r, r, r),
                             gv1=f(B, ci, r, r, r), gv2=f(B, cm, r, r, r))
    self.logits = f(B, C, 128, 128, 128)
    self.glogits = f(B, C, 128, 128, 128)
    self.skip_src = {2: "stage5", 3: "stage4", 4: "stage3", 5: "stage2"}
    self.skip_hw = {k: stage_hw[self.skip_src[k]] for k in self.skip_src}
    self.smap = {k: f(B, self.skip_hw[k][0], self.skip_hw[k][1], sk[k]) for k in sk}
    self.ray_idx = ({k: t.zeros(B, (2 * self.dec[k].r) ** 3, dtype=t.int16, device=dev) for k in sk}
                    if hasattr(self.be, "ray_sample_fwd_idx") and max(h * w for h, w in self.skip_hw.values()) < 65535 else None)
    gs_n = {k: B * sk[k] * self.skip_hw[k][0] * self.skip_hw[k][1] for k in sk}
    self.gsmap_slab = f(sum(gs_n.values()))
    self.gsmap, o = {}, 0
    for k in sk:
      self.gsmap[k] = self.gsmap_slab[o:o + gs_n[k]].view(B, sk[k], *self.skip_hw[k]); o += gs_n[k]
    self.layer_mats = f(4, B, 16)
    self._layer_scale_list = [128.0 / (2 * self.dec[k].r) for k in (2, 3, 4, 5)]
    self.layer_scales = t.tensor([[128.0 / (2 * self.dec[k].r)] * 3 + [1.0] for k in (2, 3, 4, 5)],
                                 dtype=eng.dtype, device=dev).reshape(4, 1, 1, 4)
    self.offset = f(B, 3)
    self.loss = f(1)
    self.gt = t.zeros(B, 128, 128, 128, dtype=t.int32, device=dev)
    self.side = eng.side_stream()
    use_side = self.side is not None
    self._side_ev, self._side_i = [], 0
    self._side_done = t.cuda.Event() if use_side else None
    self._ximg_ev = t.cuda.Event() if use_side else None
    self._ct_ximg = self._ct_ximg_buf = None
    self._handed_over = False
    self._g_compact = None
    self._wg_pending = []
    self._skip_ev = {k: (t.cuda.Event(), t.cuda.Event()) for k in (2, 3, 4, 5)} if use_side else None
    self._skip_bwd_ev = {k: t.cuda.Event() for k in (2, 3, 4, 5)} if use_side else None
    self._skip_bwd_done = t.cuda.Event() if use_side else None
    self._skip_async_live = False

  def _cached(self, key, fn):
    v = self._views.get(key)
    if v is None:
      v = fn()
      self._views[key] = v
    return v

  def vw(self, x: t.Tensor) -> V.View:
    return self._cached(("v", x.data_ptr(), tuple(x.shape), tuple(x.stride())), lambda: V.view_of(x))

  def s2d(self, x: t.Tensor, c1: int, r) -> V.View:
    pm = tuple(r) == (2, 2, 2)
    return self._cached(("s2d", x.data_ptr(), tuple(x.shape), tuple(x.stride()), c1, r),
                        lambda: V.space_to_depth_view(self.vw(x).channels(0, c1), r, parity_major=pm))

  def flat(self, x: t.Tensor) -> V.View:
    return self._cached(("flat", x.data_ptr(), tuple(x.shape)), lambda: V.flat_channel_view(self.vw(x)))

  probes = None

  def _probe(self, name: str, fn):
    if self.probes is None or name not in self.probes:
      return fn()
    a, b = t.cuda.Event(enable_timing=True), t.cuda.Event(enable_timing=True)
    a.record(); r = fn(); b.record()
    self.probes[name].append((a, b))
    return r

  @property
  def overlap(self) -> bool:
    return self.side is not None and self.trace is None

  def _on_side(self, after=None):
    return on_stream(self.side, after)

  def _next_handover_event(self):
    if self._side_i == len(self._side_ev):
      self._side_ev.append(t.cuda.Event())
    ev = self._side_ev[self._side_i]; self._side_i += 1
    ev.record()
    return ev

  def _stats(self, bn: BN, x: t.Tensor, S: int, sB: int, pre_relu: bool, training: bool):
    if not training:
      return
    with _lib.roctx_range("bn_stats C%d S%d" % (bn.C, S)):
      self.be.bn_stats(x, self.B, bn.C, S, sB, pre_relu, bn.gamma, bn.beta, bn.rmean, bn.rvar, bn.nbt,
                       BN_EPS, BN_MOMENTUM, True, bn.scale, bn.shift, bn.saved)

  def _bn_finalize(self, b: BN, parts: int, count: int):
    self.be.bn_finalize(parts, b.C, count, b.gamma, b.beta, b.rmean, b.rvar, b.nbt, BN_EPS, BN_MOMENTUM, b.scale, b.shift, b.saved)

  def _bn_bwd(self, b: BN, x: t.Tensor, dy: t.Tensor, dx: t.Tensor, S: int, pre_relu: bool, post_relu: bool, bias_of: Optional[Conv] = None):
    n = b.C * S
    self.be.bn_bwd(x, n, dy, n, self.B, b.C, S, pre_relu, post_relu, b.gamma, b.scale, b.shift, b.saved, dx, n, b.dgamma, b.dbeta,
                   dsum=None if bias_of is None else bias_of.dbias, ndsum=0 if bias_of is None else bias_of.n_ref)

  trace = None

  def _timed(self, label, fn):
    if _lib.ROCTX:
      with _lib.roctx_range(label):
        return fn()
    if self.trace is None:
      return fn()
    a, b = t.cuda.Event(enable_timing=True), t.cuda.Event(enable_timing=True)
    a.record(); r = fn(); b.record()
    self.trace.append((label, a, b))
    return r

  def _math(self, cv: Conv, direction: str) -> str:
    if cv.wop_kind == "e2d" and (direction == "fwd" and cv.wop_f is not None or
                                 direction == "dgrad" and cv.wop_d is not None):
      return "e2d"
    return "bf16x3" if self.eng.decoder_math == "bf16x3" and (cv.name, direction) in BF16X3_LAUNCHES else "fp32"

  conv_positions = None

  @staticmethod
  def _e2d_shape_ok(v: V.View, window) -> bool:
    S = v.D * v.H * v.W
    if S % 4:
      return False
    if tuple(window) == (1, 3, 3):
      tw = 16 if v.W % 16 == 0 else 8
      return v.D == 1 and v.W % tw == 0 and v.H % (64 // tw) == 0
    return S % 64 == 0

  @staticmethod
  def _wg2d_shape_ok(v: V.View, window) -> bool:
    return (v.D * v.H * v.W) % 32 == 0 and (tuple(window) == (1, 1, 1) or v.W % 8 == 0)

  def _conv(self, cv: Conv, x: V.View, tr, y: V.View, accumulate=False):
    g = cv.fwd
    if self.conv_positions is not None:
      self.conv_positions[cv.name] = y.D * y.H * y.W
    if cv.wop_f is not None and cv.wop_kind == "e2d" and self._e2d_shape_ok(y, g.window):
      self._timed("fwd   " + cv.name, lambda: self.be.conv2d_bf3(
          x, tr, cv.wop_f, g.npad, cv.bias, 0, y, g.window, g.pad_lo, accumulate))
      return
    self._timed("fwd   " + cv.name, lambda: self.be.conv_fwd(
        x, tr, cv.wf, g.npad, cv.bias, 0, y, g.window, g.pad_lo, 0, accumulate, boxes=(g.n_boxes, g.c_boxes),
        math=self._math(cv, "fwd"), wslab=cv.wop_f if cv.wop_kind == "slab" else None))

  def _dgrad(self, cv: Conv, dy: V.View, dx: V.View, accumulate=False):
    g = cv.dgrad
    if cv.wop_d is not None and cv.wop_kind == "e2d" and self._e2d_shape_ok(dx, g.window):
      self._timed("dgrad " + cv.name, lambda: self.be.conv2d_bf3(
          dy, None, cv.wop_d, g.npad, None, 0, dx, g.window, g.pad_lo, accumulate))
      return
    self._timed("dgrad " + cv.name, lambda: self.be.conv_fwd(
        dy, None, cv.wd, g.npad, None, 0, dx, g.window, g.pad_lo, 0, accumulate, boxes=(g.n_boxes, g.c_boxes),
        math=self._math(cv, "dgrad"), wslab=cv.wop_d if cv.wop_kind == "slab" else None))

  def _dgrad_pair(self, c1: Conv, dy1: V.View, c2: Conv, dy2: V.View, dx: V.View) -> bool:
    be = self.be
    g1, g2 = c1.dgrad, c2.dgrad
    if (getattr(be, "conv1x1_pair", None) is None or self._math(c1, "dgrad") != "fp32" or self._math(c2, "dgrad") != "fp32"
        or any(tuple(g.window) != (1, 1, 1) or any(g.pad_lo) for g in (g1, g2)) or g1.npad != g2.npad):
      return False
    return self._timed("dgrad " + c1.name + " + " + c2.name,
                       lambda: be.conv1x1_pair(dy1, c1.wd, dy2, c2.wd, g1.npad, dx))

  def _dgrad_bn_bwd(self, cv: Conv, dy: V.View, g: t.Tensor, x: t.Tensor, Cn: int, S: int, b, dx: t.Tensor, cprev: Conv) -> bool:
    be = self.be
    gvw = self.vw(g)
    fusable = (hasattr(be, "conv_dgrad_bn_bwd") and cv.wop_kind == "slab" and cv.wop_d is not None
               and self._math(cv, "dgrad") == "bf16x3")
    if not fusable:
      be.splitk_defer()
      self._dgrad(cv, dy, gvw)
      return False
    gd = cv.dgrad
    be.splitk_defer()
    return self._timed("dgrad " + cv.name, lambda: be.conv_dgrad_bn_bwd(
        dy, cv.wop_d, gd.npad, gvw, g, gd.window, gd.pad_lo, (gd.n_boxes, gd.c_boxes), x, Cn * S, self.B, Cn, S, True, b.gamma,
        b.scale, b.shift, b.saved, dx, Cn * S, b.dgamma, b.dbeta, dsum=cprev.dbias, ndsum=cprev.n_ref))

  def _wgrad_math(self, cv: Conv, dy: V.View) -> str:
    g = cv.fwd
    math = self._math(cv, "wgrad")
    if self.stem_fast and cv.name == "encoder.stage1.conv.":
      math = "stem"
    if (self.eng.encoder_e2d and g.window in ((1, 1, 1), (1, 3, 3)) and self._wg2d_shape_ok(dy, g.window)
        and (cv.name.startswith("encoder.stage") and not cv.name.startswith("encoder.stage1")
             or cv.name.startswith("decoder.rt_skip"))):
      math = "bf16x3_2d"
    if cv.ct_kind == "par" and math == "bf16x3":
      math = "ct_par"
    return math

  def _launch_wgrad(self, cv: Conv, x: V.View, tr, dy: V.View, math: str, kw: dict):
    g = cv.fwd
    with _lib.roctx_range("wgrad " + cv.name):
      self.be.conv_wgrad(x, tr, dy, cv.gwf, g.npad, g.window, g.pad_lo, False, boxes=(g.n_boxes, g.c_boxes), math=math, **kw)

  def _wgrad(self, cv: Conv, x: V.View, tr, dy: V.View, here: bool = False):
    math = self._wgrad_math(cv, dy)
    kw = self._ximg_kw(math)
    if here:
      return self._launch_wgrad(cv, x, tr, dy, math, kw)
    if not self.overlap:
      return self._timed("wgrad " + cv.name, lambda: self._launch_wgrad(cv, x, tr, dy, math, kw))
    if cv.name.startswith("encoder."):
      self._wg_pending.append((cv, x, tr, dy, math, kw))
      return
    if self._handed_over:
      self._handed_over = False
      self._side_i = max(self._side_i, 1)
      ev = None
    else:
      ev = self._next_handover_event()
    with self._on_side(after=ev):
      self._launch_wgrad(cv, x, tr, dy, math, kw)

  def _ximg_kw(self, math: str) -> dict:
    if math != "ct_par" or self._ct_ximg is None:
      return _NO_KW
    img, self._ct_ximg = self._ct_ximg, None
    return {"ximg": img}

  def _flush_wgrads(self, then=None):
    if not self._wg_pending and then is None:
      return
    with self._on_side(after=self._next_handover_event()):
      for args in self._wg_pending:
        self._launch_wgrad(*args)
      if then is not None:
        then()
    self._wg_pending = []

  def _join_side(self):
    self._flush_wgrads()
    if self._side_i:
      self._side_done.record(self.side)
      t.cuda.current_stream().wait_event(self._side_done)
      self._side_i = 0

  def _bias_grad(self, cv: Conv, dy: t.Tensor, S: int, sB: int):
    self.be.bias_grad(dy, self.B, cv.n_ref, S, sB, cv.dbias)

  def forward(self, image_u8: t.Tensor, v2s: t.Tensor, offset: t.Tensor, training: bool) -> t.Tensor:
    self._skip_async_live = bool(training and self.overlap)
    if self._skip_async_live:
      self._decoder_inputs(v2s, offset)
    self.forward_encoder(image_u8, training)
    try:
      return self.forward_decoder(v2s, offset, training)
    finally:
      self._skip_async_live = False

  def _decoder_inputs(self, v2s: t.Tensor, offset: t.Tensor):
    B = self.B
    if (hasattr(self.be, "decoder_inputs") and v2s.dtype == self.layer_mats.dtype and offset.dtype == self.offset.dtype
        and v2s.is_contiguous() and offset.is_contiguous() and v2s.device == self.layer_mats.device):
      self.be.decoder_inputs(v2s, offset, self._layer_scale_list, self.layer_mats, self.offset)
      return
    self.offset.copy_(offset)
    v = v2s.to(self.layer_mats.dtype).reshape(1, B, 4, 4)
    self.layer_mats.copy_((v * self.layer_scales).reshape(4, B, 16))

  def _skip_fwd(self, k: int):
    eng, be, B = self.eng, self.be, self.B
    d = self.dec[k]
    out = self.dec[k + 1].u
    ft = self.feat[self.skip_src[k]]
    (hh, ww), ro = self.skip_hw[k], 2 * d.r
    be.fill_offset_channels(ft, B, ft.stride(0), ft.shape[2] * ft.shape[3], ft.shape[1] - 3, self.offset)
    self._conv(eng.convs[f"decoder.rt_skip_{k}.compress_channels."], self.vw(ft), None,
               self.vw(self.smap[k].permute(0, 3, 1, 2)))
    if self.ray_idx is not None and self.training:
      self._probe(f"ray_sample_fwd_{ro}", lambda: be.ray_sample_fwd_idx(
          self.smap[k], self.smap[k].stride(0), B, eng.skip_ch[k], hh, ww, self.layer_mats[k - 2],
          self.offset, out[:, d.cout:], out.stride(0), ro, ro, ro, self.ray_idx[k], map_sC=1, map_sP=eng.skip_ch[k]))
    else:
      self._probe(f"ray_sample_fwd_{ro}", lambda: be.ray_sample_fwd(
          self.smap[k], self.smap[k].stride(0), B, eng.skip_ch[k], hh, ww, self.layer_mats[k - 2],
          self.offset, out[:, d.cout:], out.stride(0), ro, ro, ro, map_sC=1, map_sP=eng.skip_ch[k]))

  def _skip_fwd_async(self, stage: str):
    k = {v: kk for kk, v in self.skip_src.items()}[stage]
    ready, done = self._skip_ev[k]
    ready.record()
    with self._on_side(after=ready):
      self._skip_fwd(k)
      done.record(self.side)

  def forward_encoder(self, image_u8: t.Tensor, training: bool):
    if tuple(image_u8.shape) != tuple(self.in_image.shape):
      raise ValueError(f"plan for images {tuple(self.in_image.shape)}, got {tuple(image_u8.shape)}")
    eng, be, B = self.eng, self.be, self.B
    self.generation += 1
    if training and self.side is not None and (eng.dgrad_dirty or eng.weights_dirty):
      dec_later = eng.weights_dirty
      if dec_later:
        eng.pack_weights("enc_early")
      eng._pack_ev.record()
      with self._on_side(after=eng._pack_ev):
        if dec_later:
          eng.pack_weights("enc_late")
          eng._enc_late_packed.record(self.side)
          eng.pack_weights("dec")
          eng._dec_packed.record(self.side)
        if eng.dgrad_dirty:
          eng.pack_dgrad_weights()
        be.zero(eng.gpacked)
        eng._dgrad_packed.record(self.side)
      eng._dgrad_pack_pending = True
      eng._dec_pack_pending = dec_later
      eng._enc_late_pending = dec_later
      eng._gpacked_zeroed = True
    elif eng.weights_dirty:
      eng.pack_weights()
    cv, bn = eng.convs, eng.bns
    self.training = training
    if not training:
      eng.bn_eval_affine()
    be.preprocess(image_u8, self.img)
    c1 = cv["encoder.stage1.conv."]
    b1 = bn["encoder.stage1_part2.bn."]
    H1, W1 = self.stem_hw
    if self.stem_fast:
      if self.conv_positions is not None:
        self.conv_positions[c1.name] = H1 * W1
      parts = self._timed("fwd   " + c1.name, lambda: be.stem_conv_fwd(self.img, c1.wf, c1.bias, self.y1, training))
      if training:
        self._bn_finalize(b1, parts, B * H1 * W1)
    else:
      self._conv(c1, self.s2d(self.img, 3, (1, 2, 2)), None, self.vw(self.y1))
      self._stats(b1, self.y1, H1 * W1, 64 * H1 * W1, False, training)
    be.maxpool_fwd(self.y1, b1.scale, b1.shift, B, 64, H1, W1, self.p1, self.p1_arg)
    cur = self.p1
    for blk in self.blocks:
      if eng._enc_late_pending and blk.stage != "stage2":
        t.cuda.current_stream().wait_event(eng._enc_late_packed)
        eng._enc_late_pending = False
      cur = self._block_fwd(blk, cur, training)
      if blk.final and self._skip_async_live:
        self._skip_fwd_async(blk.stage)
    f5 = self.feat["stage5"]
    S5 = f5.shape[2] * f5.shape[3]
    be.relu_mean_fwd(f5, B, 2048, S5, f5.stride(0), self.avg)

  def forward_decoder(self, v2s: t.Tensor, offset: t.Tensor, training: bool) -> t.Tensor:
    eng, be, B = self.eng, self.be, self.B
    cv, bn = eng.convs, eng.bns
    self.generation += 1
    if eng._dec_pack_pending:
      t.cuda.current_stream().wait_event(eng._dec_packed)
      eng._dec_pack_pending = False
    skip_async = self._skip_async_live
    if not skip_async:
      self._decoder_inputs(v2s, offset)
    L = eng.latent
    s = eng.store
    be.linear_fwd(self.avg, s.view("decoder.stage_0.weight"), s.view("decoder.stage_0.bias"), B, 2048, L, self.z0, L + 3)
    be.fill_offset_channels(self.z0, B, L + 3, 1, L, self.offset)
    b = bn["decoder.stage_1.b1."]
    self._stats(b, self.z0, 1, L + 3, True, training)
    zv = self.vw(self.z0.view(B, L + 3, 1, 1, 1))
    self._conv(cv["decoder.stage_1.t1."], zv, Transform(b.scale, b.shift, pre_relu=True), self.flat(self.dec[2].u))
    for k in range(2, 7):
      d = self.dec[k]
      S = d.r ** 3
      p = f"decoder.stage_{k}."
      b1_, b2_ = bn[p + "b1."], bn[p + "b2."]
      tr1, tr2 = Transform(b1_.scale, b1_.shift, pre_relu=True), Transform(b2_.scale, b2_.shift, pre_relu=True)
      if skip_async and k == 3:
        t.cuda.current_stream().wait_event(self._skip_ev[2][1])
      self._stats(b1_, d.u, S, d.cin * S, True, training)
      if training:
        be.splitk_defer()
      cc = cv[p + "c1."]
      if (training and self.dec_stats_fused and cc.wop_kind == "slab" and cc.wop_f is not None and self._math(cc, "fwd") == "bf16x3"
          and self.trace is None):
        gq = cc.fwd
        parts = self._probe(f"conv3d_stage{k}_c1_fwd", lambda: self._timed("fwd   " + cc.name, lambda: be.conv_fwd_stats(
            self.vw(d.u), tr1, cc.wop_f, gq.npad, cc.bias, 0, self.vw(d.w), gq.window, gq.pad_lo, (gq.n_boxes, gq.c_boxes), d.cmid, True)))
      else:
        parts = 0
        self._probe(f"conv3d_stage{k}_c1_fwd", lambda: self._conv(cc, self.vw(d.u), tr1, self.vw(d.w)))
      if parts > 0:
        self._bn_finalize(b2_, parts, B * S)
      else:
        self._stats(b2_, d.w, S, d.cmid * S, True, training)
      out = self.dec[k + 1].u if k < 6 else self.logits
      ct = cv[p + "t1."]
      self._ct_ximg = None
      if training and self.overlap and ct.ct_kind == "par" and hasattr(be, "convt_ximage") and self._math(ct, "wgrad") == "bf16x3":
        self._ximg_ev.record()
        with self._on_side(after=self._ximg_ev):
          self._ct_ximg = self._ct_ximg_buf = be.convt_ximage(d.w, tr2, self._ct_ximg_buf)
      if ct.ct_f is not None and self._math(ct, "fwd") == "bf16x3":
        if self.conv_positions is not None:
          self.conv_positions[ct.name] = S
        self._probe(f"conv3d_stage{k}_t1_fwd", lambda: self._timed("fwd   " + ct.name, lambda: be.convt_par_fwd(
            d.w, tr2, ct.ct_f, ct.bias, out, d.cout, resident=ct.ct_kind == "res")))
      else:
        ov = self.s2d(out, d.cout, (2, 2, 2))
        self._probe(f"conv3d_stage{k}_t1_fwd", lambda: self._conv(ct, self.vw(d.w), tr2, ov))
      if k < 6 and not skip_async:
        self._skip_fwd(k)
    if training:
      be.add_i64(eng.store.nbt, eng.store.nbt.numel(), 1)
    return self.logits

  def _block_fwd(self, blk: EncBlock, cur: t.Tensor, training: bool) -> t.Tensor:
    eng, be, B = self.eng, self.be, self.B
    cv, bn = eng.convs, eng.bns
    p = blk.prefix
    S = blk.h * blk.w
    f1, f2, f3 = blk.f
    if blk.stride == 2:
      if blk.xs_filled:
        blk.xs_filled = False
      else:
        be.stride2_gather(cur, blk.xs)
      xin = self.vw(blk.xs)
    else:
      xin = self.vw(cur)
    ba, bb, bc = bn[p + "op_a.bn."], bn[p + "op_b.bn."], bn[p + "op_c.bn."]
    defer = be.splitk_defer if training else (lambda: None)
    defer()
    self._conv(cv[p + "op_a.conv."], xin, None, self.vw(blk.ya))
    self._stats(ba, blk.ya, S, f1 * S, False, training)
    defer()
    self._conv(cv[p + "op_b.conv."], self.vw(blk.ya), Transform(ba.scale, ba.shift, post_relu=True), self.vw(blk.yb))
    self._stats(bb, blk.yb, S, f2 * S, False, training)
    if blk.final:
      pre, sB_pre = self.feat[blk.stage], self.feat[blk.stage].stride(0)
    else:
      pre, sB_pre = None, 0
    fused_tail = training and hasattr(be, "bn_stats_tail")
    res, rsc, rsh = cur, None, None
    def shortcut():
      bs = bn[p + "shortcut.bn."]
      defer()
      self._conv(cv[p + "shortcut.conv."], xin, None, self.vw(blk.ys))
      self._stats(bs, blk.ys, S, f3 * S, False, training)
      return blk.ys, bs.scale, bs.shift
    if blk.down and fused_tail:
      res, rsc, rsh = shortcut()
    defer()
    self._conv(cv[p + "op_c.conv."], self.vw(blk.yb), Transform(bb.scale, bb.shift, post_relu=True), self.vw(blk.yc))
    if fused_tail:
      nxt = blk.xs_next
      with _lib.roctx_range("bn_stats_tail C%d S%d" % (bc.C, S)):
        be.bn_stats_tail(blk.yc, B, f3, S, f3 * S, bc.gamma, bc.beta, bc.rmean, bc.rvar, bc.nbt, BN_EPS, BN_MOMENTUM,
                         True, bc.scale, bc.shift, bc.saved, res, rsc, rsh, f3 * S, pre, sB_pre, blk.out, f3 * S, True,
                         y2=nxt.xs if nxt is not None else None, W=blk.w)
      if nxt is not None:
        nxt.xs_filled = True
    else:
      self._stats(bc, blk.yc, S, f3 * S, False, training)
      if blk.down:
        res, rsc, rsh = shortcut()
      be.affine_add_relu(blk.yc, bc.scale, bc.shift, res, rsc, rsh, B, f3, S, f3 * S, f3 * S, pre, sB_pre, blk.out, f3 * S, True)
    blk.inp = cur
    return blk.out

  def _grads_ready(self, label: str, hook):
    if hook is None:
      self._flush_wgrads()
      return
    eng = self.eng
    i = [b[0] for b in eng.grad_buckets].index(label)
    _, lo, hi = eng.grad_buckets[i]
    tiles = eng.bucket_unpack_tiles(i)
    def run():
      if tiles[0].numel() or tiles[3].numel():
        self.be.copy_tiles(eng.gpacked, eng.store.grads, tiles, reverse=True)
      hook(eng.store.grads[lo:hi])
    if not self.overlap:
      return run()
    return self._flush_wgrads(then=run)

  def backward(self, glogits: t.Tensor, grad_hook=None):
    eng, be, B = self.eng, self.be, self.B
    cv, bn = eng.convs, eng.bns
    assert self.training, "backward needs a training-mode forward"
    if eng._dgrad_pack_pending:
      t.cuda.current_stream().wait_event(eng._dgrad_packed)
      eng._dgrad_pack_pending = False
    elif eng.dgrad_dirty:
      eng.pack_dgrad_weights()
    if not eng._gpacked_zeroed:
      be.zero(eng.gpacked)
    eng._gpacked_zeroed = False
    overlap = self.overlap
    if overlap:
      with self._on_side():
        be.zero(self.gsmap_slab)
      if grad_hook is None:
        grad_hook = _no_exchange
    else:
      be.zero(self.gsmap_slab)
    L = eng.latent
    g_out = glogits
    for k in range(6, 1, -1):
      d = self.dec[k]
      S, So = d.r ** 3, (2 * d.r) ** 3
      p = f"decoder.stage_{k}."
      b1_, b2_ = bn[p + "b1."], bn[p + "b2."]
      ctot = g_out.shape[1]
      if k < 6:
        if overlap:
          self._skip_bwd_ev[k].record()
          with self._on_side(after=self._skip_bwd_ev[k]):
            self._skip_bwd(k, g_out, on_side=True)
            if k == 2:
              self._skip_bwd_done.record(self.side)
          self._handed_over = True
        else:
          self._skip_bwd(k, g_out, on_side=False)
      ct = cv[p + "t1."]
      gv = self.s2d(g_out, d.cout, (2, 2, 2))
      tr2 = Transform(b2_.scale, b2_.shift, pre_relu=True)
      self._wgrad(ct, self.vw(d.w), tr2, gv)
      self._handed_over = False
      if k == 6:
        if overlap:
          with self._on_side():
            self._bias_grad(ct, g_out, So, ctot * So)
        else:
          self._bias_grad(ct, g_out, So, ctot * So)
      cc = cv[p + "c1."]
      if ct.ct_d is not None and self._math(ct, "dgrad") == "bf16x3":
        self._timed("dgrad " + ct.name, lambda: be.convt_par_dgrad(g_out, d.cout, ct.ct_d, d.gv2, False, resident=ct.ct_kind == "res"))
        ct_done = False
      else:
        ct_done = self._dgrad_bn_bwd(ct, gv, d.gv2, d.w, d.cmid, S, b2_, d.gw, cc)
      if not ct_done:
        self._bn_bwd(b2_, d.w, d.gv2, d.gw, S, True, False, bias_of=cc)
      tr1 = Transform(b1_.scale, b1_.shift, pre_relu=True)
      self._wgrad(cc, self.vw(d.u), tr1, self.vw(d.gw))
      cprev = cv[f"decoder.stage_{k - 1}.t1."]
      if not self._dgrad_bn_bwd(cc, self.vw(d.gw), d.gv1, d.u, d.cin, S, b1_, d.gu, cprev):
        self._bn_bwd(b1_, d.u, d.gv1, d.gu, S, True, False, bias_of=cprev)
      g_out = d.gu
      if k == 3:
        self._grads_ready("decoder.stage_3.", grad_hook)
    c1 = cv["decoder.stage_1.t1."]
    b = bn["decoder.stage_1.b1."]
    zv = self.vw(self.z0.view(B, L + 3, 1, 1, 1))
    gv = self.flat(g_out)
    self._wgrad(c1, zv, Transform(b.scale, b.shift, pre_relu=True), gv)
    self._dgrad(c1, gv, self.vw(self.gv0.view(B, L + 3, 1, 1, 1)))
    self._bn_bwd(b, self.z0, self.gv0, self.gz0, 1, True, False)
    s = eng.store
    be.linear_bwd(self.avg, s.view("decoder.stage_0.weight"), self.gz0, L + 3, B, 2048, L, self.gavg,
                  s.view("decoder.stage_0.weight", grad=True), s.view("decoder.stage_0.bias", grad=True))
    self._grads_ready("decoder.stage_0.", grad_hook)
    if overlap:
      t.cuda.current_stream().wait_event(self._skip_bwd_done)
    f5, g5 = self.feat["stage5"], self.gfeat["stage5"]
    last = self.blocks[-1]
    S5 = f5.shape[2] * f5.shape[3]
    be.relu_mean_bwd(f5, self.gavg, B, 2048, S5, f5.stride(0), last.gpre, 2048 * S5, False)
    be.affine_add_relu(last.gpre, None, None, g5, None, None, B, 2048, S5, 2048 * S5, g5.stride(0),
                       None, 0, last.gpre, 2048 * S5, False)
    g_in = None
    for blk in reversed(self.blocks):
      g_in = self._block_bwd(blk, g_in)
      self._flush_wgrads()
      if blk.prefix in GRAD_BUCKET_LABELS:
        self._grads_ready(blk.prefix, grad_hook)
    b1 = bn["encoder.stage1_part2.bn."]
    H1, W1 = self.stem_hw
    be.maxpool_bwd(g_in, self.p1_arg, B, 64, H1, W1, self.gy1)
    cs = cv["encoder.stage1.conv."]
    self._bn_bwd(b1, self.y1, self.gy1, self.gy1b, H1 * W1, False, False, bias_of=cs)
    self._wgrad(cs, self.s2d(self.img, 3, (1, 2, 2)), None, self.vw(self.gy1b))
    self._grads_ready("", grad_hook)
    self._join_side()
    if grad_hook is None:
      be.copy_tiles(eng.gpacked, eng.store.grads, eng.unpack_tiles, reverse=True)

  def _ray_bwd(self, k: int, g_out: t.Tensor):
    d, gm = self.dec[k], self.gsmap[k]
    ro, (hh, ww) = 2 * d.r, self.skip_hw[k]
    if self.ray_idx is not None:
      self.be.ray_sample_bwd_idx(g_out[:, d.cout:], g_out.stride(0), self.B, self.eng.skip_ch[k], ro, ro, ro,
                                 self.ray_idx[k], gm, gm.stride(0), hh, ww, False)
      return
    self.be.ray_sample_bwd(g_out[:, d.cout:], g_out.stride(0), self.B, self.eng.skip_ch[k], ro, ro, ro,
                           self.layer_mats[k - 2], self.offset, gm, gm.stride(0), hh, ww, False)

  def _skip_bwd(self, k: int, g_out: t.Tensor, on_side: bool):
    (hh, ww), ns, gm = self.skip_hw[k], self.eng.skip_ch[k], self.gsmap[k]
    self._ray_bwd(k, g_out)
    cs = self.eng.convs[f"decoder.rt_skip_{k}.compress_channels."]
    self._wgrad(cs, self.vw(self.feat[self.skip_src[k]]), None, self.vw(gm), here=on_side)
    self._bias_grad(cs, gm, hh * ww, ns * hh * ww)
    self._dgrad(cs, self.vw(gm), self.vw(self.gfeat[self.skip_src[k]]))

  def _block_bwd(self, blk: EncBlock, g_out: Optional[t.Tensor]) -> t.Tensor:
    eng, be, B = self.eng, self.be, self.B
    cv, bn = eng.convs, eng.bns
    p = blk.prefix
    S = blk.h * blk.w
    f1, f2, f3 = blk.f
    ba, bb, bc = bn[p + "op_a.bn."], bn[p + "op_b.bn."], bn[p + "op_c.bn."]
    gpre = blk.gpre
    cc, cb, ca = cv[p + "op_c.conv."], cv[p + "op_b.conv."], cv[p + "op_a.conv."]
    fused_head = g_out is not None and hasattr(be, "bn_bwd_head")
    gc, self._g_compact = self._g_compact, None
    if gc is not None and not fused_head:
      be.stride2_scatter(gc, g_out)
      gc = None
    if blk.final:
      act, sB_act, g2, sB_g2 = (self.feat[blk.stage], self.feat[blk.stage].stride(0),
                                self.gfeat[blk.stage], self.gfeat[blk.stage].stride(0))
    else:
      act, sB_act, g2, sB_g2 = blk.out, f3 * S, None, 0
    if fused_head:
      be.bn_bwd_head(blk.yc, f3 * S, gpre, f3 * S, g_out, f3 * S, act, sB_act, g2, sB_g2, B, f3, S, bc.gamma, bc.scale,
                     bc.shift, bc.saved, blk.gyc, f3 * S, bc.dgamma, bc.dbeta, dsum=cc.dbias, ndsum=cc.n_ref,
                     g_compact=gc, W=blk.w)
    else:
      if g_out is not None:
        be.relu_bwd_add(g_out, act, g2, B, f3, S, f3 * S, sB_act, sB_g2, gpre, f3 * S)
      self._bn_bwd(bc, blk.yc, gpre, blk.gyc, S, False, False, bias_of=cc)
    trb = Transform(bb.scale, bb.shift, post_relu=True)
    tra = Transform(ba.scale, ba.shift, post_relu=True)
    self._wgrad(cc, self.vw(blk.yb), trb, self.vw(blk.gyc))
    be.splitk_defer()
    self._dgrad(cc, self.vw(blk.gyc), self.vw(blk.gab))
    self._bn_bwd(bb, blk.yb, blk.gab, blk.gyb, S, False, True, bias_of=cb)
    self._wgrad(cb, self.vw(blk.ya), tra, self.vw(blk.gyb))
    be.splitk_defer()
    self._dgrad(cb, self.vw(blk.gyb), self.vw(blk.gaa))
    self._bn_bwd(ba, blk.ya, blk.gaa, blk.gya, S, False, True, bias_of=ca)
    xin = self.vw(blk.xs) if blk.stride == 2 else self.vw(blk.inp)
    self._wgrad(ca, xin, None, self.vw(blk.gya))
    if blk.down:
      bs = bn[p + "shortcut.bn."]
      csn = cv[p + "shortcut.conv."]
      self._bn_bwd(bs, blk.ys, gpre, blk.gys, S, False, False, bias_of=csn)
      self._wgrad(csn, xin, None, self.vw(blk.gys))
      gin = blk.gin
      gv = self.vw(blk.gxs) if blk.stride == 2 else self.vw(gin)
      if not self._dgrad_pair(ca, self.vw(blk.gya), csn, self.vw(blk.gys), gv):
        self._dgrad(ca, self.vw(blk.gya), gv)
# ... 10 lines not shown
```

include/corenet_hip.h:

```cpp
#ifndef CORENET_HIP_H_
#define CORENET_HIP_H_

#include <stddef.h>
#include <stdint.h>

#ifdef __cplusplus
extern "C" {
#endif

#define CRN_OK 0
#define CRN_EINVAL (-1)
#define CRN_ENOMEM (-2)
#define CRN_ENOCONV (-3)

typedef void* crnStream;

typedef struct {
  float* base;
  int32_t B, C, D, H, W;
  int64_t sB, sC;
  const int32_t* chan_off;
  int32_t sD, sH, sW;
} crnView;

// ... 168 lines not shown
int crn_bias_grad(const float* dy, int B, int C, int64_t S, int64_t sB, float* db,
                  int accumulate, double* workspace ,
                  size_t workspace_bytes, crnStream s);

int crn_batch_renorm_stats(const float* x, int B, int C, int64_t S, int64_t sB, int pre_relu,
                           const float* gamma, const float* beta,
                           float* running_mean, float* running_var,
                           const int64_t* num_batches_tracked ,
                           float eps, float momentum, int training,
                           float* scale, float* shift, float* saved ,
                           double* workspace, size_t workspace_bytes, crnStream s);
size_t crn_batch_renorm_workspace_bytes(int C);
int crn_batch_renorm_stats_tail(const float* x, int B, int C, int64_t S, int64_t sB,
                                const float* gamma, const float* beta, float* running_mean, float* running_var,
                                const int64_t* num_batches_tracked, float eps, float momentum, int training,
                                float* scale, float* shift, float* saved, double* workspace, size_t workspace_bytes,
                                const float* r, const float* rscale, const float* rshift, int64_t sB_r,
                                float* y_pre, int64_t sB_pre, float* y, int64_t sB_y, int relu,
                                float* y2, int W, crnStream s);

int crn_batch_renorm_eval_affine(const float* params, const float* buffers, const int32_t* table,
                                 int n, float eps, float* scale, float* shift, crnStream s);

int crn_batch_renorm_bwd(const float* x, int64_t sB_x, const float* dy, int64_t sB_dy,
                         int B, int C, int64_t S, int pre_relu, int post_relu,
                         const float* gamma, const float* scale, const float* shift,
                         const float* saved, float* dx, int64_t sB_dx,
                         float* dgamma, float* dbeta, int accumulate,
                         float* dsum, int ndsum,
                         double* workspace, size_t workspace_bytes, crnStream s);

int crn_batch_renorm_bwd_apply(const float* x, int64_t sB_x, const float* dy, int64_t sB_dy,
                               int B, int C, int64_t S, int pre_relu,
                               const float* gamma, const float* scale, const float* shift,
                               const float* saved, float* dx, int64_t sB_dx,
                               float* dgamma, float* dbeta, int accumulate,
                               float* dsum, int ndsum,
                               double* workspace, size_t workspace_bytes, int nparts, crnStream s);

int crn_batch_renorm_bwd_head(const float* x, int64_t sB_x, float* dy, int64_t sB_dy,
                              const float* g, int64_t sB_g, const float* act, int64_t sB_act,
                              const float* g2 , int64_t sB_g2,
                              int B, int C, int64_t S, const float* gamma, const float* scale, const float* shift,
                              const float* saved, float* dx, int64_t sB_dx, float* dgamma, float* dbeta,
                              int accumulate, float* dsum, int ndsum,
                              double* workspace, size_t workspace_bytes, const float* g_compact, int W, crnStream s);

int crn_affine_add_relu(const float* x, const float* scale, const float* shift,
                        const float* r, const float* rscale, const float* rshift,
                        int B, int C, int64_t S, int64_t sB_x, int64_t sB_r,
                        float* y_pre, int64_t sB_pre, float* y, int64_t sB_y,
                        int relu, crnStream s);

int crn_relu_bwd_add(const float* dy, const float* y_pre, const float* dy2,
                     int B, int C, int64_t S, int64_t sB_dy, int64_t sB_pre, int64_t sB_dy2,
                     float* dx, int64_t sB_dx, crnStream s);

size_t crn_stem_conv_parts(int B, int H, int W);
int crn_stem_conv_fwd(const float* img, int B, int H, int W, const float* w_packed, const float* bias,
                      float* y, double* stats_ws , size_t ws_bytes, crnStream s);
int crn_stem_conv_wgrad(const float* img, int B, int H, int W, const float* dy, float* dw_packed, crnStream s);
int crn_batch_renorm_finalize(const double* ws, int nparts, int C, double count,
                              const float* gamma, const float* beta, float* running_mean, float* running_var,
                              const int64_t* nbt, float eps, float momentum,
                              float* scale, float* shift, float* saved, crnStream s);

int crn_preprocess_caffe(const uint8_t* img, int B, int H, int W, float* out, crnStream s);
int crn_bn_relu_maxpool_fwd(const float* x, const float* scale, const float* shift,
                            int B, int C, int H, int W, float* y, int32_t* argmax, crnStream s);
int crn_bn_relu_maxpool_bwd(const float* dy, const int32_t* argmax, int B, int C, int H, int W,
                            float* dx_bn , crnStream s);
int crn_relu_mean_fwd(const float* x_pre, int B, int C, int64_t S, int64_t sB, float* avg, crnStream s);
int crn_linear_fwd(const float* x, const float* w, const float* bias, int B, int K, int N,
                   float* y, int ldy, crnStream s);
int crn_linear_bwd(const float* x, const float* w, const float* dy, int lddy, int B, int K, int N,
                   float* dx, float* dw, float* db, crnStream s);
int crn_relu_mean_bwd(const float* x_pre, const float* davg, int B, int C, int64_t S, int64_t sB,
                      float* dx, int64_t sB_dx, int accumulate, crnStream s);
int crn_stride2_gather(const float* x, float* y, int B, int C, int h, int w, int hin, int win, crnStream s);
int crn_stride2_scatter(const float* dy, float* dx, int B, int C, int h, int w, int hin, int win, crnStream s);
int crn_fill_offset_channels(float* x, int B, int64_t sB, int64_t S, int c0,
                             const float* offset, crnStream s);

int crn_decoder_inputs(const float* v2s, const float* offset, int B, int nscales, const float* scales,
                       float* layer_mats, float* offset_out, crnStream s);

int crn_ray_sample_fwd(const float* map, int64_t map_sB, int64_t map_sC, int64_t map_sP,
                       int B, int C, int h, int w, const float* matrix, const float* offset,
                       float* out, int64_t out_sB, int D, int H, int W, crnStream s);
int crn_ray_sample_bwd(const float* dout, int64_t dout_sB, int B, int C, int D, int H, int W,
                       const float* matrix, const float* offset,
                       float* dmap, int64_t dmap_sB, int h, int w, int zero_first, crnStream s);
int crn_ray_sample_fwd_idx(const float* map, int64_t map_sB, int64_t map_sC, int64_t map_sP,
                           int B, int C, int h, int w, const float* matrix, const float* offset,
                           float* out, int64_t out_sB, int D, int H, int W, uint16_t* idx, crnStream s);
int crn_ray_project(const float* matrix, const float* offset, int B, int D, int H, int W, int h, int w,
                    uint16_t* idx, crnStream s);
int crn_ray_sample_bwd_idx(const float* dout, int64_t dout_sB, int B, int C, int D, int H, int W,
                           const uint16_t* idx, float* dmap, int64_t dmap_sB, int h, int w, int zero_first,
                           crnStream s);

int crn_loss_fwd_bwd(int kind, const float* logits, const int32_t* gt, const float* weights,
                     int B, int C, int64_t S, float* loss, float* dlogits, float grad_scale,
                     void* workspace, size_t workspace_bytes, crnStream s);
size_t crn_loss_workspace_bytes(int B, int C);
const int* crn_loss_status_ptr(void* workspace, int B);

int crn_argmax_confusion(const float* logits, const int32_t* gt, int B, int C, int64_t S,
                         int32_t* labels, int64_t* cm, crnStream s);

int crn_softmax_superres(const float* logits, int m, int B, int C, int D, int H, int W, float* out,
                         crnStream s);

#define CRN_EVAL_MAX_CLASSES 32
#define CRN_EVAL_MAX_BINS 64
int crn_eval_labels(const float* scores, const int32_t* gt, const int32_t* scene_class, int B, int C, int K, int D, int H,
                    int W, int m, int n, int32_t* labels, int64_t* cm, int32_t* bad, crnStream s);
int crn_eval_labels_cpu(const float* scores, const int32_t* gt, const int32_t* scene_class, int B, int C, int K, int D, int H,
                        int W, int m, int n, int32_t* labels, int64_t* cm, int32_t* bad, int num_threads);

#define CRN_SCORE_MAX_ENTRIES 2048
#define CRN_SCORE_MAX_NBINS 256
#define CRN_SCORE_CHUNK 8192
int crn_eval_scores_tiles(int32_t* out3);
int crn_eval_scores(const float* scores, int from_logits, const int32_t* gt, const int32_t* scene_class, int B, int C, int K,
                    int D, int H, int W, int m, int n, int nbins, int64_t* table, int64_t* sq, int64_t* bad, crnStream s);
int crn_eval_scores_cpu(const float* scores, int from_logits, const int32_t* gt, const int32_t* scene_class, int B, int C,
                        int K, int D, int H, int W, int m, int n, int nbins, int64_t* table, int64_t* sq, int64_t* bad,
                        int num_threads);
int crn_score_softmax(const float* logits, int B, int C, int64_t S, float* out, crnStream s);
int crn_score_softmax_cpu(const float* logits, int B, int C, int64_t S, float* out, int num_threads);

int crn_adam_step(float* param, const float* grad, float* exp_avg, float* exp_avg_sq,
                  int64_t n, float lr, float beta1, float beta2, float eps,
                  float grad_scale, int step, crnStream s);
int crn_adam_set_hyper(float* hyper, float lr, float beta1, float beta2, float eps, float grad_scale,
                       int step, crnStream s);
int crn_adam_step_hyper(float* param, const float* grad, float* exp_avg, float* exp_avg_sq,
                        int64_t n, const float* hyper, crnStream s);

int crn_bf3_gather_image(const float* src, const int32_t* table, int n_entries, void* dst, crnStream s);
int crn_convt_s2k7_fwd_bf3(const float* x, int64_t x_sB, int B, int D, int H, int W, const crnInTransform* tr,
                           const void* wimg, const float* bias, float* y, int64_t y_sB, int64_t y_sC, int Cout, crnStream s);
int crn_convt_s2k7_dgrad_bf3(const float* dy, int64_t dy_sB, int64_t dy_sC, int Cout, int B, int D, int H, int W,
                             const void* wimg, float* dx, int64_t dx_sB, int accumulate, crnStream s);
int crn_convt_s2k7_c2_fwd_bf3(const float* x, int64_t x_sB, int B, int D, int H, int W, const crnInTransform* tr,
                              const void* wimg, const float* bias, float* y, int64_t y_sB, int64_t y_sC, int Cout, crnStream s);
int crn_convt_s2k7_c2_dgrad_bf3(const float* dy, int64_t dy_sB, int64_t dy_sC, int Cout, int B, int D, int H, int W,
                                const void* wimg, float* dx, int64_t dx_sB, int accumulate, crnStream s);
int crn_convt_s2k7_wgrad_bf3(const float* x, int64_t x_sB, int B, int D, int H, int W, const crnInTransform* tr,
                             const float* dy, int64_t dy_sB, int64_t dy_sC, int Cout, float* dw, int Npad, int zero_first,
                             const void* ximg, crnStream s);
size_t crn_convt_s2k7_ximage_bytes(int B, int D, int H, int W);
int crn_convt_s2k7_ximage(const float* x, int64_t x_sB, int B, int D, int H, int W, const crnInTransform* tr,
                          void* img, size_t img_bytes, crnStream s);

int crn_fill_voxels(const void* grid, void* out, int dtype, int N, int D, int H, int W,
                    void* workspace, size_t workspace_bytes, crnStream s);
size_t crn_fill_voxels_workspace_bytes(int N, int D, int H, int W);
int crn_fill_voxels_strided(const void* grid, const int64_t* grid_strides, void* out, const int64_t* out_strides,
                            int dtype, int N, int D, int H, int W, void* workspace, size_t workspace_bytes, crnStream s);

int crn_fill_voxels_cpu(const void* grid, void* out, int dtype, int N, int D, int H, int W,
                        int num_threads);

#define CRN_MC_MAX_OBJECT_CELLS ((int64_t)1 << 29)
size_t crn_marching_cubes_workspace_bytes(int N, int D, int H, int W);
int crn_marching_cubes_count(const float* grid, const int64_t* strides, int N, int D, int H, int W, float level,
                             void* workspace, size_t workspace_bytes, int64_t* counts, crnStream s);
int crn_marching_cubes_emit(const float* grid, const int64_t* strides, int N, int D, int H, int W, float level,
                            const float* matrices, void* workspace, size_t workspace_bytes, float* vertices,
                            float* normals, int32_t* faces, crnStream s);
int crn_box_filter(const float* in, const int64_t* strides, float* out, int N, int D, int H, int W, int k,
                   void* workspace, size_t workspace_bytes, crnStream s);
int crn_marching_cubes_cpu(const float* grid, const int64_t* strides, int N, int D, int H, int W, float level,
                           const float* matrices, int64_t* counts, float* vertices, float* normals, int32_t* faces,
                           int num_threads);
int crn_box_filter_cpu(const float* in, const int64_t* strides, float* out, int N, int D, int H, int W, int k,
                       int num_threads);

#define CRN_RENDER_TILE 16
typedef struct {
  float vp[16];
  float light[3], cam[3], light_color[3], ambient_light[3], clear[3];
  int32_t cull, normal_mode, t0, t1, inst0, pad[4];
} crnRenderImage;
int crn_render_bin(const float* triangles, const crnRenderImage* images, int I, int H, int W, int max_len,
// ... 207 lines not shown
```

Measured before the change: 1.215 billion.

## Fuse decoder head linear+BN and loss finalize into fewer kernels

Adds fused kernels for the decoder head: forward linear, offset fill and batch-renorm stats run in one launch, and the backward BN, linear weight/bias grads and relu-mean/residual add are merged into two kernels. It also folds the loss finalize reduction and the num_batches_tracked increment into the loss pass-2 kernel, which removes the separate add_i64 launch. The aim is to cut launch count and small-kernel latency in a launch-bound training step. The cost is some redundant reduction work per block and serial per-thread loops over the batch.

```diff
diff --git a/corenet_amd/_lib.py b/corenet_amd/_lib.py
--- a/corenet_amd/_lib.py
+++ b/corenet_amd/_lib.py
@@ -159,6 +159,10 @@
     "crn_ray_project": [vp, vp, i32, i32, i32, i32, i32, i32, vp, vp],
     "crn_ray_sample_bwd_idx": [vp, i64, i32, i32, i32, i32, i32, vp, vp, i64, i32, i32, i32, vp],
     "crn_loss_fwd_bwd": [i32, vp, vp, vp, i32, i32, i64, vp, vp, f32, vp, sz, vp],
+    "crn_loss_fwd_bwd_fused": [i32, vp, vp, vp, i32, i32, i64, vp, vp, f32, vp, sz, vp, i32, vp],
+    "crn_decoder_head_fwd": [vp, vp, vp, vp, i32, i32, i32, vp, i32, vp, vp, vp, vp, vp, f32, f32, vp, vp, vp, vp],
+    "crn_decoder_head_bwd_params": [vp, vp, i32, i32, i32, i32, vp, vp, vp, vp, vp, vp, vp, vp, vp, vp, vp],
+    "crn_decoder_head_bwd_data": [vp, i32, vp, i32, i32, i32, vp, i64, vp, i64, i64, vp, i64, vp],
     "crn_argmax_confusion": [vp, vp, i32, i32, i64, vp, vp, vp],
     "crn_softmax_superres": [vp, i32, i32, i32, i32, i32, i32, vp, vp],
     "crn_eval_labels": [vp, vp, vp, i32, i32, i32, i32, i32, i32, i32, i32, vp, vp, vp, vp],
diff --git a/corenet_amd/backend.py b/corenet_amd/backend.py
--- a/corenet_amd/backend.py
+++ b/corenet_amd/backend.py
@@ -385,6 +385,25 @@
     self.lib.crn_linear_bwd(ptr(x), ptr(w), ptr(dy), lddy, B, K, N, ptr(dx), ptr(dw), ptr(db),
                             _lib.stream())
 
+  @staticmethod
+  def decoder_head_ok(B, L) -> bool:
+    return 1 <= B <= 64 and L + 3 >= 64
+
+  def decoder_head_fwd(self, avg, w, bias, offset, B, K, L, z0, pre_relu, gamma, beta, rmean, rvar, nbt, eps, momentum,
+                       scale, shift, saved):
+    self.lib.crn_decoder_head_fwd(ptr(avg), ptr(w), ptr(bias), ptr(offset), B, K, L, ptr(z0), int(pre_relu), ptr(gamma),
+                                  ptr(beta), ptr(rmean), ptr(rvar), ptr(nbt), eps, momentum, ptr(scale), ptr(shift),
+                                  ptr(saved), _lib.stream())
+
+  def decoder_head_bwd_params(self, z0, gv0, B, K, L, pre_relu, gamma, scale, shift, saved, gz0, dgamma, dbeta, avg, dw, db):
+    self.lib.crn_decoder_head_bwd_params(ptr(z0), ptr(gv0), B, K, L, int(pre_relu), ptr(gamma), ptr(scale), ptr(shift),
+                                         ptr(saved), ptr(gz0), ptr(dgamma), ptr(dbeta), ptr(avg), ptr(dw), ptr(db),
+                                         _lib.stream())
+
+  def decoder_head_bwd_data(self, gz0, lddy, w, B, K, L, f5, sB_f5, g5, sB_g5, S, gpre, sB_gpre):
+    self.lib.crn_decoder_head_bwd_data(ptr(gz0), lddy, ptr(w), B, K, L, ptr(f5), sB_f5, ptr(g5), sB_g5, S, ptr(gpre),
+                                       sB_gpre, _lib.stream())
+
   def stride2_gather(self, x, y):
     B, Cn, h, w = y.shape
     self.lib.crn_stride2_gather(ptr(x), ptr(y), B, Cn, h, w, x.shape[2], x.shape[3], _lib.stream())
@@ -428,6 +447,13 @@
     ws = self.workspace("loss", n, logits.device)
     self.lib.crn_loss_fwd_bwd(kind, ptr(logits), ptr(gt_i32), ptr(weights), B, Cn, S, ptr(loss), ptr(dlogits),
                               grad_scale, ptr(ws), n, _lib.stream())
+
+  def loss_fwd_bwd_fused(self, kind, logits, gt_i32, B, Cn, S, loss, dlogits, grad_scale=1.0, weights=None, counters=None):
+    n = self.lib.crn_loss_workspace_bytes(B, Cn)
+    ws = self.workspace("loss", n, logits.device)
+    self.lib.crn_loss_fwd_bwd_fused(kind, ptr(logits), ptr(gt_i32), ptr(weights), B, Cn, S, ptr(loss), ptr(dlogits),
+                                    grad_scale, ptr(ws), n, ptr(counters), 0 if counters is None else counters.numel(),
+                                    _lib.stream())
 
   def loss_labels_in_range(self, B, Cn, device) -> bool:
     n = self.lib.crn_loss_workspace_bytes(B, Cn)
diff --git a/corenet_amd/csrc/batch_renorm.hip b/corenet_amd/csrc/batch_renorm.hip
--- a/corenet_amd/csrc/batch_renorm.hip
+++ b/corenet_amd/csrc/batch_renorm.hip
@@ -548,6 +548,108 @@
   }
 }
 
+constexpr int kHeadMaxB = 64;
+
+__global__ __launch_bounds__(kThreads) void decoder_head_fwd_kernel(
+    const float* avg, const float* w, const float* bias, const float* offset, int B, int K, int L, float* z0, int pre_relu,
+    const float* gamma, const float* beta, float* running_mean, float* running_var, const int64_t* nbt, float eps,
+    float momentum, float* scale, float* shift, float* saved) {
+  __shared__ double red[kThreads / 64];
+  __shared__ float zs[kHeadMaxB];
+  const int j = blockIdx.x, C = L + 3;
+  const int lane = threadIdx.x & 63, wave = threadIdx.x >> 6;
+  const BnChannelIn cin = bn_channel_in(j, gamma, beta, running_mean, running_var, nbt);
+  if (j < L) {
+    for (int b = wave; b < B; b += kThreads / 64) {
+      float s = 0.f;
+#pragma unroll 8
+      for (int k = lane; k < K; k += 64) s += avg[(int64_t)b * K + k] * w[(int64_t)j * K + k];
+      s = crn_wave_sum(s);
+      if (lane == 0) {
+        const float v = s + (bias ? bias[j] : 0.f);
+        zs[b] = v;
+        z0[(int64_t)b * C + j] = v;
+      }
+    }
+  } else if ((int)threadIdx.x < B) {
+    const float v = offset[threadIdx.x * 3 + (j - L)];
+    zs[threadIdx.x] = v;
+    z0[(int64_t)threadIdx.x * C + j] = v;
+  }
+  __syncthreads();
+  double s1 = 0.0, s2 = 0.0;
+  if (threadIdx.x == 0)
+    for (int b = 0; b < B; ++b) bn_acc(zs[b], pre_relu, s1, s2);
+  const double t1 = crn_block_sum(s1, red);
+  const double t2 = crn_block_sum(s2, red);
+  if (threadIdx.x == 0)
+    bn_finalize_channel(j, C, t1, t2, (double)B, cin, running_mean, running_var, eps, momentum, scale, shift, saved);
+}
+
+__global__ __launch_bounds__(kThreads) void decoder_head_bwd_params_kernel(
+    const float* z0, const float* gv0, int B, int C, int L, int K, int pre_relu, const float* gamma, const float* scale,
+    const float* shift, const float* saved, float* gz0, float* dgamma, float* dbeta, const float* avg, float* dw, float* db) {
+  __shared__ double red[kThreads / 64];
+  __shared__ float sm[2];
+  __shared__ float gs[kHeadMaxB];
+  const int c = blockIdx.x;
+  const BnBwdChannel ch = bn_bwd_channel(c, C, scale, shift, saved);
+  double s1 = 0.0, s2 = 0.0;
+  if (threadIdx.x == 0)
+    for (int b = 0; b < B; ++b) bn_bwd_acc(z0[(int64_t)b * C + c], gv0[(int64_t)b * C + c], pre_relu, 0, ch, s1, s2);
+  const double t1 = crn_block_sum(s1, red);
+  const double t2 = crn_block_sum(s2, red);
+  if (threadIdx.x == 0)
+    bn_bwd_store_grad(bn_bwd_close(t1, t2, (double)B, saved[2 * C + c], saved[3 * C + c], sm), c, dgamma, dbeta, 0);
+  __syncthreads();
+  const float mg = sm[0], mgx = sm[1];
+  const float k = gamma[c] * saved[2 * C + c] * ch.rstd;
+  if ((int)threadIdx.x < B) {
+    const int b = threadIdx.x;
+    const float o = bn_bwd_dx(z0[(int64_t)b * C + c], gv0[(int64_t)b * C + c], pre_relu, 0, ch, k, mg, mgx);
+    gz0[(int64_t)b * C + c] = o;
+    gs[b] = o;
+  }
+  if (c >= L) return;
+  __syncthreads();
+  for (int kk = threadIdx.x; kk < K; kk += kThreads) {
+    float s = 0.f;
+    for (int b = 0; b < B; ++b) s += gs[b] * avg[(int64_t)b * K + kk];
+    dw[(int64_t)c * K + kk] = s;
+  }
+  if (threadIdx.x == 0 && db) {
+    float t = 0.f;
+    for (int b = 0; b < B; ++b) t += gs[b];
+    db[c] = t;
+  }
+}
+
+constexpr int kHeadCT = 32;
+__global__ __launch_bounds__(kThreads) void decoder_head_bwd_data_kernel(
+    const float* gz0, int lddy, const float* w, int K, int N, const float* f5, int64_t sBf, const float* g5, int64_t sBg,
+    int S, float* gpre, int64_t sBo) {
+  __shared__ float ga[kHeadCT];
+  const int b = blockIdx.y, c0 = blockIdx.x * kHeadCT;
+  const int nc = min(kHeadCT, K - c0);
+  if ((int)threadIdx.x < nc) {
+    const int kcol = c0 + threadIdx.x;
+    float s = 0.f;
+#pragma unroll 16
+    for (int n = 0; n < N; ++n) s += gz0[(int64_t)b * lddy + n] * w[(int64_t)n * K + kcol];
+    ga[threadIdx.x] = s;
+  }
+  __syncthreads();
+  const int64_t base = (int64_t)c0 * S;
+  const float* pf = f5 + (int64_t)b * sBf + base;
+  const float* pg = g5 + (int64_t)b * sBg + base;
+  float* po = gpre + (int64_t)b * sBo + base;
+  const float one = 1.f, zero = 0.f;
+  for (int e = threadIdx.x; e < nc * S; e += kThreads) {
+    const float g = pf[e] > 0.f ? ga[e / S] / (float)S : 0.f;
+    po[e] = g * one + zero + (pg[e] * one + zero);
+  }
+}
+
 inline bool owner_form(int64_t S, int C, int B) {
   return C >= 64 && (int64_t)B * S <= 65536 && ((int64_t)B * S <= 16384 || C >= 256);
 }
@@ -1026,3 +1128,42 @@
   }
   return bias_grad_ordered(dy, B, C, S, sB, nsplit_for(S, C, B), db, accumulate, ws, ws_bytes, st);
 }
+
+extern "C" int crn_decoder_head_fwd(const float* avg, const float* w, const float* bias, const float* offset, int B, int K,
+                                    int L, float* z0, int pre_relu, const float* gamma, const float* beta,
+                                    float* running_mean, float* running_var, const int64_t* nbt, float eps, float momentum,
+                                    float* scale, float* shift, float* saved, crnStream stream) {
+  CRN_ENTRY(stream);
+  if (B < 1 || B > kHeadMaxB || K < 1 || L < 1 || !owner_form(1, L + 3, B)) return CRN_EINVAL;
+  if (!avg || !w || !offset || !z0 || !gamma || !beta || !running_mean || !running_var || !nbt || !scale || !shift || !saved)
+    return CRN_EINVAL;
+  hipLaunchKernelGGL(decoder_head_fwd_kernel, dim3(L + 3), dim3(kThreads), 0, (hipStream_t)stream, avg, w, bias, offset, B, K, L,
+                     z0, pre_relu, gamma, beta, running_mean, running_var, nbt, eps, momentum, scale, shift, saved);
+  CRN_CHECK_LAUNCH();
+  return CRN_OK;
+}
+
+extern "C" int crn_decoder_head_bwd_params(const float* z0, const float* gv0, int B, int K, int L, int pre_relu,
+                                           const float* gamma, const float* scale, const float* shift, const float* saved,
+                                           float* gz0, float* dgamma, float* dbeta, const float* avg, float* dw, float* db,
+                                           crnStream stream) {
+  CRN_ENTRY(stream);
+  if (B < 1 || B > kHeadMaxB || K < 1 || L < 1 || !owner_form(1, L + 3, B)) return CRN_EINVAL;
+  if (!z0 || !gv0 || !gamma || !scale || !shift || !saved || !gz0 || !dgamma || !dbeta || !avg || !dw) return CRN_EINVAL;
+  hipLaunchKernelGGL(decoder_head_bwd_params_kernel, dim3(L + 3), dim3(kThreads), 0, (hipStream_t)stream, z0, gv0, B, L + 3, L, K,
+                     pre_relu, gamma, scale, shift, saved, gz0, dgamma, dbeta, avg, dw, db);
+  CRN_CHECK_LAUNCH();
+  return CRN_OK;
+}
+
+extern "C" int crn_decoder_head_bwd_data(const float* gz0, int lddy, const float* w, int B, int K, int L, const float* f5,
+                                         int64_t sB_f5, const float* g5, int64_t sB_g5, int64_t S, float* gpre, int64_t sB_gpre,
+                                         crnStream stream) {
+  CRN_ENTRY(stream);
+  if (B < 1 || B > 65535 || K < 1 || L < 1 || lddy < L || S < 1 || S > (1 << 24)) return CRN_EINVAL;
+  if (!gz0 || !w || !f5 || !g5 || !gpre) return CRN_EINVAL;
+  hipLaunchKernelGGL(decoder_head_bwd_data_kernel, dim3(crn_cdiv(K, kHeadCT), B), dim3(kThreads), 0, (hipStream_t)stream, gz0, lddy,
+                     w, K, L, f5, sB_f5, g5, sB_g5, (int)S, gpre, sB_gpre);
+  CRN_CHECK_LAUNCH();
+  return CRN_OK;
+}
diff --git a/corenet_amd/csrc/losses.hip b/corenet_amd/csrc/losses.hip
--- a/corenet_amd/csrc/losses.hip
+++ b/corenet_amd/csrc/losses.hip
@@ -63,19 +63,26 @@
   }
 }
 
-__global__ __launch_bounds__(1024) void loss_finalize_kernel(const double* part, int nblk, int B, int64_t S, int kind,
-                                                            float grad_scale, float* loss, float* coef, int* bad_label) {
-  __shared__ double sums[64 * kNQ];
+__device__ __forceinline__ void loss_reduce_pairs(const double* part, int nblk, int B, double* sums) {
   const int lane = threadIdx.x & 63, wave = threadIdx.x >> 6;
   for (int pair = wave; pair < B * kNQ; pair += (int)(blockDim.x >> 6)) {
     const int b = pair / kNQ, k = pair - b * kNQ;
+    const double* p = part + (int64_t)b * nblk * kNQ + k;
+    double v[8];
+#pragma unroll
+    for (int u = 0; u < 8; ++u) { const int i = lane + 64 * u; v[u] = i < nblk ? p[(int64_t)i * kNQ] : 0.0; }
     double s = 0.0;
-    for (int i = lane; i < nblk; i += 64) s += part[((int64_t)b * nblk + i) * kNQ + k];
+#pragma unroll
+    for (int u = 0; u < 8; ++u) s += v[u];
+    for (int i = lane + 512; i < nblk; i += 64) s += p[(int64_t)i * kNQ];
     s = crn_wave_sum(s);
     if (lane == 0) sums[pair] = s;
   }
-  __syncthreads();
-  if (threadIdx.x != 0) return;
+}
+
+struct LossHead { float L, kfg, kag, kx; int bad; };
+template <typename F>
+__device__ __forceinline__ LossHead loss_combine(const double* sums, int B, int64_t S, int kind, float grad_scale, F per_sample) {
   double iou_fg = 0.0, iou_ag = 0.0, xs = 0.0, nbad = 0.0;
   for (int b = 0; b < B; ++b) {
     const double* q = sums + b * kNQ;
@@ -84,7 +91,7 @@
     const float iag = (float)q[2], uag = (float)q[3] == 0.f ? 1.f : (float)q[3];
     iou_fg += (double)(ifg / ufg); iou_ag += (double)(iag / uag);
     xs += q[4];
-    coef[4 + b * 4 + 0] = ifg; coef[4 + b * 4 + 1] = ufg; coef[4 + b * 4 + 2] = iag; coef[4 + b * 4 + 3] = uag;
+    per_sample(b, ifg, ufg, iag, uag);
   }
   const float Lfg = 1.f - (float)(iou_fg / B), Lag = 1.f - (float)(iou_ag / B);
   const float X = (float)(xs / ((double)B * (double)S));
@@ -96,25 +103,28 @@
     case 3: L = X; kx = 1.f; break;
     case 4: L = (1.f + Lfg) * (1.f + X); kfg = 1.f + X; kx = 1.f + Lfg; break;
   }
-  *bad_label = nbad > 0.0 ? 1 : 0;
-  loss[0] = L;
-  coef[0] = L; coef[1] = kfg * grad_scale / B; coef[2] = kag * grad_scale / B;
-  coef[3] = kx * grad_scale / (float)((double)B * (double)S);
-}
-
-template <int CT>
-__global__ __launch_bounds__(kThreads) void loss_pass2_kernel(const float* logits, const int32_t* gt,
-                                                              const float* weights, int C, int64_t S,
-                                                              const float* coef, float* dlogits) {
-  const int b = blockIdx.y;
-  const float* lb = logits + (int64_t)b * C * S;
-  const int32_t* gb = gt + (int64_t)b * S;
-  const float* wb = weights ? weights + (int64_t)b * S : nullptr;
-  float* db = dlogits + (int64_t)b * C * S;
-  const float kfg0 = coef[1], kag0 = coef[2], kx0 = coef[3];
-  const float ifg = coef[4 + b * 4 + 0], ufg = coef[4 + b * 4 + 1];
-  const float iag = coef[4 + b * 4 + 2], uag = coef[4 + b * 4 + 3];
-  for (int64_t v = blockIdx.x * (int64_t)kThreads + threadIdx.x; v < S; v += (int64_t)gridDim.x * kThreads) {
+  return LossHead{L, kfg * grad_scale / B, kag * grad_scale / B, kx * grad_scale / (float)((double)B * (double)S),
+                  nbad > 0.0 ? 1 : 0};
+}
+
+__global__ __launch_bounds__(1024) void loss_finalize_kernel(const double* part, int nblk, int B, int64_t S, int kind,
+                                                            float grad_scale, float* loss, float* coef, int* bad_label) {
+  __shared__ double sums[64 * kNQ];
+  loss_reduce_pairs(part, nblk, B, sums);
+  __syncthreads();
+  if (threadIdx.x != 0) return;
+  const LossHead h = loss_combine(sums, B, S, kind, grad_scale, [&](int b, float ifg, float ufg, float iag, float uag) {
+    coef[4 + b * 4 + 0] = ifg; coef[4 + b * 4 + 1] = ufg; coef[4 + b * 4 + 2] = iag; coef[4 + b * 4 + 3] = uag;
+  });
+  *bad_label = h.bad;
+  loss[0] = h.L;
+  coef[0] = h.L; coef[1] = h.kfg; coef[2] = h.kag; coef[3] = h.kx;
+}
+
+template <int CT>
+__device__ __forceinline__ void loss_pass2_voxels(const float* lb, const int32_t* gb, const float* wb, float* db, int C, int64_t S,
+                                                  float kfg0, float kag0, float kx0, float ifg, float ufg, float iag, float uag) {
+  for (int64_t v = blockIdx.x * (int64_t)blockDim.x + threadIdx.x; v < S; v += (int64_t)gridDim.x * blockDim.x) {
     Soft<CT> sm;
     sm.compute(lb + v, S, C);
     int g = gb[v];
@@ -154,6 +164,49 @@
   }
 }
 
+
+template <int CT>
+__global__ __launch_bounds__(kThreads) void loss_pass2_kernel(const float* logits, const int32_t* gt,
+                                                              const float* weights, int C, int64_t S,
+                                                              const float* coef, float* dlogits) {
+  const int b = blockIdx.y;
+  const float kfg0 = coef[1], kag0 = coef[2], kx0 = coef[3];
+  const float ifg = coef[4 + b * 4 + 0], ufg = coef[4 + b * 4 + 1];
+  const float iag = coef[4 + b * 4 + 2], uag = coef[4 + b * 4 + 3];
+  loss_pass2_voxels<CT>(logits + (int64_t)b * C * S, gt + (int64_t)b * S, weights ? weights + (int64_t)b * S : nullptr,
+                        dlogits + (int64_t)b * C * S, C, S, kfg0, kag0, kx0, ifg, ufg, iag, uag);
+}
+
+constexpr int kFoldThreads = 1024;
+template <int CT>
+__global__ __launch_bounds__(kFoldThreads) void loss_pass2_fold_kernel(
+    const float* logits, const int32_t* gt, const float* weights, int C, int64_t S, const double* part, int nblk, int B, int kind,
+    float grad_scale, float* loss, float* coef, int* bad_label, int64_t* nbt, int n_nbt, float* dlogits) {
+  __shared__ double sums[64 * kNQ];
+  __shared__ float mine[7];
+  const int b = blockIdx.y;
+  const bool first = blockIdx.x == 0 && b == 0;
+  loss_reduce_pairs(part, nblk, B, sums);
+  if (first && nbt)
+    for (int i = threadIdx.x; i < n_nbt; i += kFoldThreads) nbt[i] += 1;
+  __syncthreads();
+  if (threadIdx.x == 0) {
+    const LossHead h = loss_combine(sums, B, S, kind, grad_scale, [&](int bb, float ifg, float ufg, float iag, float uag) {
+      if (bb == b) { mine[3] = ifg; mine[4] = ufg; mine[5] = iag; mine[6] = uag; }
+      if (first) { coef[4 + bb * 4 + 0] = ifg; coef[4 + bb * 4 + 1] = ufg; coef[4 + bb * 4 + 2] = iag; coef[4 + bb * 4 + 3] = uag; }
+    });
+    mine[0] = h.kfg; mine[1] = h.kag; mine[2] = h.kx;
+    if (first) {
+      *bad_label = h.bad;
+      loss[0] = h.L;
+      coef[0] = h.L; coef[1] = h.kfg; coef[2] = h.kag; coef[3] = h.kx;
+    }
+  }
+  __syncthreads();
+  loss_pass2_voxels<CT>(logits + (int64_t)b * C * S, gt + (int64_t)b * S, weights ? weights + (int64_t)b * S : nullptr,
+                        dlogits + (int64_t)b * C * S, C, S, mine[0], mine[1], mine[2], mine[3], mine[4], mine[5], mine[6]);
+}
+
 template <int CT>
 __global__ __launch_bounds__(kThreads) void argmax_confusion_kernel(const float* logits, const int32_t* gt,
                                                                     int C, int64_t S, int32_t* labels,
@@ -190,12 +243,13 @@
   return (size_t)B * 512 * kNQ * sizeof(double) + (size_t)(4 + 4 * B) * sizeof(float) + 64;
 }
 
-extern "C" int crn_loss_fwd_bwd(int kind, const float* logits, const int32_t* gt, const float* weights, int B, int C,
-                                int64_t S, float* loss, float* dlogits, float grad_scale, void* workspace,
-                                size_t workspace_bytes, crnStream stream) {
+static int loss_fwd_bwd_impl(int kind, const float* logits, const int32_t* gt, const float* weights, int B, int C,
+                             int64_t S, float* loss, float* dlogits, float grad_scale, void* workspace,
+                             size_t workspace_bytes, bool fold, int64_t* nbt, int n_nbt, crnStream stream) {
   CRN_ENTRY(stream);
   hipStream_t st = (hipStream_t)stream;
   if (kind < 0 || kind > 4 || B < 1 || B > 64 || C < 2 || C > 32 || S < 1 || !logits || !gt || !loss) return CRN_EINVAL;
+  if (nbt && n_nbt < 1) return CRN_EINVAL;
   if (workspace_bytes < crn_loss_workspace_bytes(B, C)) return CRN_ENOMEM;
   const int nblk = loss_nblk(S);
   double* part = reinterpret_cast<double*>(workspace);
@@ -207,6 +261,13 @@
   else if (C <= 16) CRN_LOSS_P1(16); else CRN_LOSS_P1(32);
 #undef CRN_LOSS_P1
   CRN_CHECK_LAUNCH();
+  if (fold && dlogits && C <= 2) {
+    dim3 fgrid(crn_cdiv(nblk, kFoldThreads / kThreads), B);
+    hipLaunchKernelGGL(loss_pass2_fold_kernel<2>, fgrid, dim3(kFoldThreads), 0, st, logits, gt, weights, C, S, part, nblk, B, kind,
+                       grad_scale, loss, coef, bad_label, nbt, n_nbt, dlogits);
+    CRN_CHECK_LAUNCH();
+    return CRN_OK;
+  }
   hipLaunchKernelGGL(loss_finalize_kernel, dim3(1), dim3(1024), 0, st, part, nblk, B, S, kind, grad_scale, loss, coef, bad_label);
   CRN_CHECK_LAUNCH();
   if (dlogits) {
@@ -216,7 +277,22 @@
 #undef CRN_LOSS_P2
     CRN_CHECK_LAUNCH();
   }
+  if (nbt) return crn_add_i64(nbt, n_nbt, 1, stream);
   return CRN_OK;
+}
+
+extern "C" int crn_loss_fwd_bwd(int kind, const float* logits, const int32_t* gt, const float* weights, int B, int C,
+                                int64_t S, float* loss, float* dlogits, float grad_scale, void* workspace,
+                                size_t workspace_bytes, crnStream stream) {
+  return loss_fwd_bwd_impl(kind, logits, gt, weights, B, C, S, loss, dlogits, grad_scale, workspace, workspace_bytes, false,
+                           nullptr, 0, stream);
+}
+
+extern "C" int crn_loss_fwd_bwd_fused(int kind, const float* logits, const int32_t* gt, const float* weights, int B, int C,
+                                      int64_t S, float* loss, float* dlogits, float grad_scale, void* workspace,
+                                      size_t workspace_bytes, int64_t* counters, int n_counters, crnStream stream) {
+  return loss_fwd_bwd_impl(kind, logits, gt, weights, B, C, S, loss, dlogits, grad_scale, workspace, workspace_bytes, true,
+                           counters, n_counters, stream);
 }
 
 extern "C" const int* crn_loss_status_ptr(void* workspace, int B) {
diff --git a/corenet_amd/model/core_net.py b/corenet_amd/model/core_net.py
--- a/corenet_amd/model/core_net.py
+++ b/corenet_amd/model/core_net.py
@@ -385,13 +385,13 @@
       if graph and graphable:
         return self._train_step_graph(plan, image, voxel_projection_matrix, voxel_sample_locations, grid, loss, lr,
                                       adam_eps, 1.0 / world_size)
-      plan.forward(image.contiguous(), voxel_projection_matrix, voxel_sample_locations, training=True)
+      fused = self._loss_fused()
+      plan.forward(image.contiguous(), voxel_projection_matrix, voxel_sample_locations, training=True, nbt_with_loss=fused)
       if grid.dtype == t.int32 and grid.device == plan.gt.device and grid.is_contiguous() and grid.shape == plan.gt.shape:
         gt = grid
       else:
         plan.gt.copy_(grid); gt = plan.gt
-      eng.be.loss_fwd_bwd(LOSS_KINDS[loss], plan.logits, gt, B, C, plan.logits[0, 0].numel(), plan.loss,
-                          plan.glogits, 1.0)
+      self._loss(fused, LOSS_KINDS[loss], plan, gt)
       if all_reduce is not None and getattr(all_reduce, "overlap", False):
         all_reduce.pushed.clear()
         step_buckets = hasattr(all_reduce, "opt_stream") and plan.overlap and all_reduce.opt_stream() is not None
@@ -420,12 +420,25 @@
       eng.adam_step(lr, adam_eps, grad_scale=1.0 / world_size)
       return plan.loss
 
+  def _loss_fused(self) -> bool:
+    eng = self.engine
+    return bool(eng.head_fused and hasattr(eng.be, "loss_fwd_bwd_fused"))
+
+  def _loss(self, fused: bool, kind: int, plan, gt: t.Tensor):
+    eng = self.engine
+    S = plan.logits[0, 0].numel()
+    if fused:
+      eng.be.loss_fwd_bwd_fused(kind, plan.logits, gt, plan.B, eng.num_classes, S, plan.loss, plan.glogits, 1.0,
+                                counters=eng.store.nbt)
+    else:
+      eng.be.loss_fwd_bwd(kind, plan.logits, gt, plan.B, eng.num_classes, S, plan.loss, plan.glogits, 1.0)
+
   def _step_body(self, plan, loss: str):
     eng = self.engine
     eng.weights_dirty = True
-    plan.forward(plan.in_image, plan.in_v2s, plan.in_off, training=True)
-    eng.be.loss_fwd_bwd(LOSS_KINDS[loss], plan.logits, plan.gt, plan.B, eng.num_classes, plan.logits[0, 0].numel(),
-                        plan.loss, plan.glogits, 1.0)
+    fused = self._loss_fused()
+    plan.forward(plan.in_image, plan.in_v2s, plan.in_off, training=True, nbt_with_loss=fused)
+    self._loss(fused, LOSS_KINDS[loss], plan, plan.gt)
     plan.backward(plan.glogits)
     eng.adam_update_from_hyper()
 
diff --git a/corenet_amd/model/engine.py b/corenet_amd/model/engine.py
--- a/corenet_amd/model/engine.py
+++ b/corenet_amd/model/engine.py
@@ -216,6 +216,7 @@
       from corenet_amd.backend import default_backend
       backend = default_backend()
     self.be = backend
+    self.head_fused = hasattr(backend, "decoder_head_fwd")
     default_math = "bf16x3" if getattr(backend, "name", "") == "hip" else "fp32"
     self.decoder_math = decoder_math or os.environ.get("CRN_DECODER_MATH", default_math)
     if self.decoder_math not in ("fp32", "bf16x3"):
@@ -587,6 +588,7 @@
     self.dec_stats_fused = hasattr(eng.be, "conv_fwd_stats")
     self.pool_hw = (H // 4, W // 4)
     self.be = eng.be
+    self._nbt_with_loss = False
     self.generation = 0
     self.graphs = {}
     self.eager_steps = 0
@@ -719,6 +721,10 @@
       self.be.bn_stats(x, self.B, bn.C, S, sB, pre_relu, bn.gamma, bn.beta, bn.rmean, bn.rvar, bn.nbt,
                        BN_EPS, BN_MOMENTUM, True, bn.scale, bn.shift, bn.saved)
 
+  def _head_fused(self, training: bool) -> bool:
+    return bool(training and self.eng.head_fused and hasattr(self.be, "decoder_head_fwd")
+                and self.be.decoder_head_ok(self.B, self.eng.latent))
+
   def _bn_finalize(self, b: BN, parts: int, count: int):
     self.be.bn_finalize(parts, b.C, count, b.gamma, b.beta, b.rmean, b.rvar, b.nbt, BN_EPS, BN_MOMENTUM, b.scale, b.shift, b.saved)
 
@@ -871,8 +877,9 @@
   def _bias_grad(self, cv: Conv, dy: t.Tensor, S: int, sB: int):
     self.be.bias_grad(dy, self.B, cv.n_ref, S, sB, cv.dbias)
 
-  def forward(self, image_u8: t.Tensor, v2s: t.Tensor, offset: t.Tensor, training: bool) -> t.Tensor:
+  def forward(self, image_u8: t.Tensor, v2s: t.Tensor, offset: t.Tensor, training: bool, nbt_with_loss: bool = False) -> t.Tensor:
     self._skip_async_live = bool(training and self.overlap)
+    self._nbt_with_loss = bool(training and nbt_with_loss)
     if self._skip_async_live:
       self._decoder_inputs(v2s, offset)
     self.forward_encoder(image_u8, training)
@@ -880,6 +887,7 @@
       return self.forward_decoder(v2s, offset, training)
     finally:
       self._skip_async_live = False
+      self._nbt_with_loss = False
 
   def _decoder_inputs(self, v2s: t.Tensor, offset: t.Tensor):
     B = self.B
@@ -985,10 +993,14 @@
       self._decoder_inputs(v2s, offset)
     L = eng.latent
     s = eng.store
-    be.linear_fwd(self.avg, s.view("decoder.stage_0.weight"), s.view("decoder.stage_0.bias"), B, 2048, L, self.z0, L + 3)
-    be.fill_offset_channels(self.z0, B, L + 3, 1, L, self.offset)
     b = bn["decoder.stage_1.b1."]
-    self._stats(b, self.z0, 1, L + 3, True, training)
+    if self._head_fused(training):
+      be.decoder_head_fwd(self.avg, s.view("decoder.stage_0.weight"), s.view("decoder.stage_0.bias"), self.offset, B, 2048, L,
+                          self.z0, True, b.gamma, b.beta, b.rmean, b.rvar, b.nbt, BN_EPS, BN_MOMENTUM, b.scale, b.shift, b.saved)
+    else:
+      be.linear_fwd(self.avg, s.view("decoder.stage_0.weight"), s.view("decoder.stage_0.bias"), B, 2048, L, self.z0, L + 3)
+      be.fill_offset_channels(self.z0, B, L + 3, 1, L, self.offset)
+      self._stats(b, self.z0, 1, L + 3, True, training)
     zv = self.vw(self.z0.view(B, L + 3, 1, 1, 1))
     self._conv(cv["decoder.stage_1.t1."], zv, Transform(b.scale, b.shift, pre_relu=True), self.flat(self.dec[2].u))
     for k in range(2, 7):
@@ -1032,7 +1044,7 @@
         self._probe(f"conv3d_stage{k}_t1_fwd", lambda: self._conv(ct, self.vw(d.w), tr2, ov))
       if k < 6 and not skip_async:
         self._skip_fwd(k)
-    if training:
+    if training and not self._nbt_with_loss:
       be.add_i64(eng.store.nbt, eng.store.nbt.numel(), 1)
     return self.logits
 
@@ -1177,19 +1189,30 @@
     gv = self.flat(g_out)
     self._wgrad(c1, zv, Transform(b.scale, b.shift, pre_relu=True), gv)
     self._dgrad(c1, gv, self.vw(self.gv0.view(B, L + 3, 1, 1, 1)))
-    self._bn_bwd(b, self.z0, self.gv0, self.gz0, 1, True, False)
     s = eng.store
-    be.linear_bwd(self.avg, s.view("decoder.stage_0.weight"), self.gz0, L + 3, B, 2048, L, self.gavg,
-                  s.view("decoder.stage_0.weight", grad=True), s.view("decoder.stage_0.bias", grad=True))
-    self._grads_ready("decoder.stage_0.", grad_hook)
+    head_fused = self._head_fused(True)
+    if head_fused:
+      be.decoder_head_bwd_params(self.z0, self.gv0, B, 2048, L, True, b.gamma, b.scale, b.shift, b.saved, self.gz0, b.dgamma,
+                                 b.dbeta, self.avg, s.view("decoder.stage_0.weight", grad=True),
+                                 s.view("decoder.stage_0.bias", grad=True))
+    else:
+      self._bn_bwd(b, self.z0, self.gv0, self.gz0, 1, True, False)
+      be.linear_bwd(self.avg, s.view("decoder.stage_0.weight"), self.gz0, L + 3, B, 2048, L, self.gavg,
+                    s.view("decoder.stage_0.weight", grad=True), s.view("decoder.stage_0.bias", grad=True))
+      self._grads_ready("decoder.stage_0.", grad_hook)
     if overlap:
       t.cuda.current_stream().wait_event(self._skip_bwd_done)
     f5, g5 = self.feat["stage5"], self.gfeat["stage5"]
     last = self.blocks[-1]
     S5 = f5.shape[2] * f5.shape[3]
-    be.relu_mean_bwd(f5, self.gavg, B, 2048, S5, f5.stride(0), last.gpre, 2048 * S5, False)
-    be.affine_add_relu(last.gpre, None, None, g5, None, None, B, 2048, S5, 2048 * S5, g5.stride(0),
-                       None, 0, last.gpre, 2048 * S5, False)
+    if head_fused:
+      be.decoder_head_bwd_data(self.gz0, L + 3, s.view("decoder.stage_0.weight"), B, 2048, L, f5, f5.stride(0), g5, g5.stride(0),
+                               S5, last.gpre, 2048 * S5)
+      self._grads_ready("decoder.stage_0.", grad_hook)
+    else:
+      be.relu_mean_bwd(f5, self.gavg, B, 2048, S5, f5.stride(0), last.gpre, 2048 * S5, False)
+      be.affine_add_relu(last.gpre, None, None, g5, None, None, B, 2048, S5, 2048 * S5, g5.stride(0),
+                         None, 0, last.gpre, 2048 * S5, False)
     g_in = None
     for blk in reversed(self.blocks):
       g_in = self._block_bwd(blk, g_in)
diff --git a/include/corenet_hip.h b/include/corenet_hip.h
--- a/include/corenet_hip.h
+++ b/include/corenet_hip.h
@@ -274,6 +274,17 @@
 int crn_fill_offset_channels(float* x, int B, int64_t sB, int64_t S, int c0,
                              const float* offset, crnStream s);
 
+int crn_decoder_head_fwd(const float* avg, const float* w, const float* bias, const float* offset, int B, int K, int L,
+                         float* z0, int pre_relu, const float* gamma, const float* beta, float* running_mean,
+                         float* running_var, const int64_t* num_batches_tracked, float eps, float momentum,
+                         float* scale, float* shift, float* saved, crnStream s);
+int crn_decoder_head_bwd_params(const float* z0, const float* gv0, int B, int K, int L, int pre_relu, const float* gamma,
+                                const float* scale, const float* shift, const float* saved, float* gz0, float* dgamma,
+                                float* dbeta, const float* avg, float* dw, float* db, crnStream s);
+int crn_decoder_head_bwd_data(const float* gz0, int lddy, const float* w, int B, int K, int L, const float* f5,
+                              int64_t sB_f5, const float* g5, int64_t sB_g5, int64_t S, float* gpre, int64_t sB_gpre,
+                              crnStream s);
+
 int crn_decoder_inputs(const float* v2s, const float* offset, int B, int nscales, const float* scales,
                        float* layer_mats, float* offset_out, crnStream s);
 
@@ -295,6 +306,9 @@
 int crn_loss_fwd_bwd(int kind, const float* logits, const int32_t* gt, const float* weights,
                      int B, int C, int64_t S, float* loss, float* dlogits, float grad_scale,
                      void* workspace, size_t workspace_bytes, crnStream s);
+int crn_loss_fwd_bwd_fused(int kind, const float* logits, const int32_t* gt, const float* weights,
+                           int B, int C, int64_t S, float* loss, float* dlogits, float grad_scale,
+                           void* workspace, size_t workspace_bytes, int64_t* counters, int n_counters, crnStream s);
 size_t crn_loss_workspace_bytes(int B, int C);
 const int* crn_loss_status_ptr(void* workspace, int B);
 
```

Measured after the change: 1.215 billion, median of 2. About the same (+0.0%).
